# Quyans/GOI-Hyperplane

Hardware: AMD Instinct MI355X
Metric: training views/sec (rasterizer fwd+bwd), 1M Gaussians @1600x1056 RGB+16-d feat (higher is better)
Workload: dtype f32

## Files before the change

### goi_hyperplane_amd/_C.py

```python
from __future__ import annotations

import collections
import ctypes as C
import os
import threading
import warnings
import weakref

import torch

from . import _lib
from ._lib import ALLOC_FN, GoiRasterScene


_EXT = {"mod": None, "tried": False, "want": os.environ.get("GOI_BINDING", "compiled").strip().lower()}
_EMPTY = torch.Tensor([])


def _ext():
    if _EXT.get("error") is not None:
        raise _EXT["error"]
    if not _EXT["tried"]:
        _EXT["tried"] = True
        path = os.path.join(os.path.dirname(_lib.LIB_PATH), "_goi_C.so")
# ... 756 lines not shown
        alloc = _BinningAllocator(dev)
        n = lib.goi_raster_forward(C.byref(sc), _ptr(geom), _ptr(img), alloc.cb, None, _ptr(out_color), _ptr(out_sem),
                                   _ptr(out_depth), _ptr(out_alpha), _ptr(radii), _stream(dev))
        if alloc.error is not None:
            raise alloc.error
        if n < 0:
            raise RuntimeError(_lib.last_error())
        if P > 0:
            SPECULATION_STATS["exact_frames"] += 1
            _note_count(dev, P, n, _tiles(H, W))
    return n, out_color, out_sem, out_depth, out_alpha, radii, geom, alloc.tensor, img


def _backward_impl(background, means3D, radii, colors, semantics, scales, rotations, scale_modifier,
                                 cov3D_precomp, viewmatrix, projmatrix, tan_fovx, tan_fovy, dL_dout_color,
                                 dL_dout_semantic, dL_dout_depth, dL_dout_alpha, sh, degree, campos, geomBuffer, R,
                                 binningBuffer, imageBuffer, alphas, debug, sh_factored=False, accumulate_into=None):
    lib = _lib.load()
    dev = _check_device(means3D)
    ext = _ext()
    if ext is not None:
        R_layout, lazy_binning = _layout_of(R)
        return ext.backward_ex(background, means3D, radii, _e(colors), semantics, _e(scales), _e(rotations),
                               float(scale_modifier), _e(cov3D_precomp), viewmatrix, projmatrix, float(tan_fovx),
                               float(tan_fovy), dL_dout_color, dL_dout_semantic, dL_dout_depth, dL_dout_alpha, _e(sh),
                               int(degree), campos, geomBuffer, R_layout,
                               binningBuffer if lazy_binning is None else lazy_binning, imageBuffer, alphas, bool(debug),
                               bool(sh_factored), _scratch_instances(R, R_layout), accumulate_into)
    if accumulate_into is not None:
        raise RuntimeError("accumulate_into needs the compiled binding (python -m goi_hyperplane_amd.build)")
    P = int(means3D.size(0))
    H, W = int(alphas.size(-2)), int(alphas.size(-1))
    S = int(semantics.size(1))
    M = 0 if (sh is None or sh.numel() == 0) else int(sh.size(1))
    sh_factored = bool(sh_factored) and M > 0
    f32 = dict(dtype=torch.float32, device=dev)
    with torch.cuda.device(dev):
        sections = (("means3D", (P, 3)), ("sh", (P, 0 if sh_factored else M, 3)), ("semantics", (P, S)),
                    ("opacity", (P, 1)), ("scales", (P, 3)), ("rotations", (P, 4)))
        offs, total = {}, 0
        for name, shape in sections:
            offs[name] = total
            n = 1
            for d in shape:
                n *= d
            total += (n + 63) // 64 * 64
        flat = torch.empty((total,), **f32)

        def view(name, shape):
            n = 1
            for d in shape:
                n *= d
            return flat[offs[name]:offs[name] + n].view(shape)
        dL_dmeans3D = view("means3D", (P, 3))
        dL_dsh = None if sh_factored else view("sh", (P, M, 3))
        dL_dsemantics = view("semantics", (P, S))
        dL_dopacity = view("opacity", (P, 1))
        dL_dscales = view("scales", (P, 3))
        dL_drotations = view("rotations", (P, 4))
        del flat
        dL_dmeans2D = torch.empty((P, 3), **f32)
        dL_dcolors = torch.empty((P, 3), **f32)
        dL_ddepths = torch.empty((P, 1), **f32)
        dL_dconic = torch.empty((P, 2, 2), **f32)
        dL_dcov3D = torch.empty((P, 6), **f32)
        if P != 0:
            ten = dict(bg=_prep(background, "background", dev), means3D=_prep(means3D, "means3D", dev),
                       sh=_prep(sh, "sh", dev), colors=_prep(colors, "colors_precomp", dev),
                       semantics=_prep(semantics, "semantics", dev), scales=_prep(scales, "scales", dev),
                       rotations=_prep(rotations, "rotations", dev), cov3D=_prep(cov3D_precomp, "cov3D_precomp", dev),
                       viewmatrix=_prep(viewmatrix, "viewmatrix", dev), projmatrix=_prep(projmatrix, "projmatrix", dev),
                       campos=_prep(campos, "campos", dev), radii=_prep(radii, "radii", dev, torch.int32),
                       alphas=_prep(alphas, "alphas", dev), g_c=_prep(dL_dout_color, "dL_dout_color", dev),
                       g_s=_prep(dL_dout_semantic, "dL_dout_semantic", dev),
                       g_d=_prep(dL_dout_depth, "dL_dout_depth", dev), g_a=_prep(dL_dout_alpha, "dL_dout_alpha", dev))
            sc = _scene(P, S, H, W, ten["bg"], ten["means3D"], ten["sh"], ten["colors"], ten["semantics"], None,
                        ten["scales"], ten["rotations"], scale_modifier, ten["cov3D"], ten["viewmatrix"],
                        ten["projmatrix"], tan_fovx, tan_fovy, degree, ten["campos"], False, debug)
            R_layout, lazy_binning = _layout_of(R)
            if lazy_binning is not None:
                binningBuffer = lazy_binning
            R_scratch = _scratch_instances(R, R_layout)
            scratch = _backward_scratch(lib.goi_raster_backward_scratch_bytes(R_scratch or R_layout, S), dev)
            r = lib.goi_raster_backward3(
                C.byref(sc), R_layout, R_scratch, 0, _ptr(geomBuffer), _ptr(binningBuffer), _ptr(imageBuffer), _ptr(ten["radii"]),
                _ptr(ten["alphas"]), _ptr(ten["g_c"]), _ptr(ten["g_s"]), _ptr(ten["g_d"]), _ptr(ten["g_a"]),
                _ptr(dL_dmeans2D), _ptr(dL_dconic), _ptr(dL_dopacity), _ptr(dL_dcolors), _ptr(dL_dsemantics),
                _ptr(dL_ddepths), _ptr(dL_dmeans3D), _ptr(dL_dcov3D), _ptr(dL_dsh), _ptr(dL_dscales),
                _ptr(dL_drotations), _ptr(scratch), None, _stream(dev))
            if r < 0:
                raise RuntimeError(_lib.last_error())
    return (dL_dmeans2D, dL_dcolors, dL_dsemantics, dL_dopacity, dL_dmeans3D, dL_dcov3D, dL_dsh, dL_dscales,
            dL_drotations)


def rasterize_gaussians_backward(background, means3D, radii, colors, semantics, scales, rotations, scale_modifier,
                                 cov3D_precomp, viewmatrix, projmatrix, tan_fovx, tan_fovy, dL_dout_color,
                                 dL_dout_semantic, dL_dout_depth, dL_dout_alpha, sh, degree, campos, geomBuffer, R,
                                 binningBuffer, imageBuffer, alphas, debug):
    return _backward_impl(background, means3D, radii, colors, semantics, scales, rotations, scale_modifier, cov3D_precomp, viewmatrix, projmatrix, tan_fovx, tan_fovy, dL_dout_color, dL_dout_semantic, dL_dout_depth, dL_dout_alpha, sh, degree, campos, geomBuffer, R, binningBuffer, imageBuffer, alphas, debug)


def rasterize_gaussians_backward_accumulate(accumulate_into, *args):
    return _backward_impl(*args, accumulate_into=accumulate_into)


def rasterize_gaussians_backward_sh_factored(background, means3D, radii, colors, semantics, scales, rotations, scale_modifier,
                                 cov3D_precomp, viewmatrix, projmatrix, tan_fovx, tan_fovy, dL_dout_color,
                                 dL_dout_semantic, dL_dout_depth, dL_dout_alpha, sh, degree, campos, geomBuffer, R,
                                 binningBuffer, imageBuffer, alphas, debug):
    return _backward_impl(background, means3D, radii, colors, semantics, scales, rotations, scale_modifier, cov3D_precomp, viewmatrix, projmatrix, tan_fovx, tan_fovy, dL_dout_color, dL_dout_semantic, dL_dout_depth, dL_dout_alpha, sh, degree, campos, geomBuffer, R, binningBuffer, imageBuffer, alphas, debug, sh_factored=True)


def sh_grad_from_views(means3D, campos, gcol, degree, M):
    lib = _lib.load()
    dev = _check_device(means3D)
    P, V = int(means3D.size(0)), int(campos.size(0))
    if tuple(gcol.shape) != (V, P, 3):
        raise ValueError(f"gcol must be [V={V}, P={P}, 3], got {tuple(gcol.shape)}")
    with torch.cuda.device(dev):
        out = torch.empty((P, int(M), 3), dtype=torch.float32, device=dev)
        if P and V:
            m, c, g = _prep(means3D, "means3D", dev), _prep(campos, "campos", dev), _prep(gcol, "gcol", dev)
            if lib.goi_raster_sh_grad_from_views(P, int(degree), int(M), V, _ptr(m), _ptr(c), _ptr(g), _ptr(out), _stream(dev)) < 0:
                raise RuntimeError(_lib.last_error())
        elif P:
            out.zero_()
    return out


def rasterize_gaussians_backward_semantics(background, means3D, radii, semantics, viewmatrix, projmatrix, tan_fovx,
                                           tan_fovy, dL_dout_semantic, campos, geomBuffer, R, binningBuffer,
                                           imageBuffer, alphas, sh_degree=0, debug=False):
    lib = _lib.load()
    dev = _check_device(means3D)
    ext = _ext()
    if ext is not None:
        R_layout, lazy_binning = _layout_of(R)
        return ext.backward_semantics(background, means3D, radii, semantics, viewmatrix, projmatrix, float(tan_fovx),
                                      float(tan_fovy), dL_dout_semantic, campos, geomBuffer, R_layout,
                                      binningBuffer if lazy_binning is None else lazy_binning, imageBuffer, alphas,
                                      int(sh_degree), bool(debug))
    P = int(means3D.size(0))
    S = int(dL_dout_semantic.size(0))
    H, W = int(dL_dout_semantic.size(1)), int(dL_dout_semantic.size(2))
    with torch.cuda.device(dev):
        dL_dsemantics = torch.empty((P, S), dtype=torch.float32, device=dev)
        if P != 0:
            ten = dict(bg=_prep(background, "background", dev), means3D=_prep(means3D, "means3D", dev),
                       semantics=_prep(semantics, "semantics", dev), viewmatrix=_prep(viewmatrix, "viewmatrix", dev),
                       projmatrix=_prep(projmatrix, "projmatrix", dev), campos=_prep(campos, "campos", dev),
                       radii=_prep(radii, "radii", dev, torch.int32), alphas=_prep(alphas, "alphas", dev),
                       g_s=_prep(dL_dout_semantic, "dL_dout_semantic", dev))
            sc = _scene(P, S, H, W, ten["bg"], ten["means3D"], None, ten["means3D"], ten["semantics"], None,
                        None, None, 1.0, ten["means3D"], ten["viewmatrix"], ten["projmatrix"], tan_fovx, tan_fovy,
                        sh_degree, ten["campos"], False, debug)
            R_layout, lazy_binning = _layout_of(R)
            if lazy_binning is not None:
                binningBuffer = lazy_binning
            scratch = _backward_scratch(lib.goi_raster_backward_scratch_bytes(R_layout, S), dev)
            r = lib.goi_raster_backward_semantics(C.byref(sc), R_layout, _ptr(geomBuffer), _ptr(binningBuffer),
                                                  _ptr(imageBuffer), _ptr(ten["radii"]), _ptr(ten["alphas"]),
                                                  _ptr(ten["g_s"]), _ptr(dL_dsemantics), _ptr(scratch), _stream(dev))
            if r < 0:
                raise RuntimeError(_lib.last_error())
    return dL_dsemantics


def rasterize_gaussians_trace(background, means3D, colors, img_sem, opacity, scales, rotations, scale_modifier,
                              cov3D_precomp, viewmatrix, projmatrix, tan_fovx, tan_fovy, image_height, image_width, sh,
                              degree, campos, prefiltered, debug):
    lib = _lib.load()
# ... 115 lines not shown
```

### goi_hyperplane_amd/_lib.py

```python
from __future__ import annotations

import ctypes as C
import os

_HERE = os.path.dirname(os.path.abspath(__file__))
LIB_PATH = os.path.join(_HERE, "lib", "libgoi_raster.so")

ABI_VERSION = 6

STAGES = ("preprocess", "depth_sort", "scan", "emit", "tile_sort", "ranges", "blend_fwd", "blend_bwd",
          "preprocess_bwd")


class GoiRasterScene(C.Structure):
    _fields_ = [
        ("P", C.c_int), ("D", C.c_int), ("M", C.c_int), ("S", C.c_int), ("W", C.c_int), ("H", C.c_int),
        ("bg", C.c_void_p), ("means3D", C.c_void_p), ("shs", C.c_void_p), ("colors_precomp", C.c_void_p),
        ("semantics", C.c_void_p), ("opacities", C.c_void_p), ("scales", C.c_void_p),
        ("scale_modifier", C.c_float), ("rotations", C.c_void_p), ("cov3D_precomp", C.c_void_p),
        ("viewmatrix", C.c_void_p), ("projmatrix", C.c_void_p), ("campos", C.c_void_p),
        ("tan_fovx", C.c_float), ("tan_fovy", C.c_float), ("prefiltered", C.c_int), ("debug", C.c_int),
    ]


ALLOC_FN = C.CFUNCTYPE(C.c_void_p, C.c_void_p, C.c_size_t)

SYMBOLS = {
    "goi_raster_abi_version": (C.c_int, []),
    "goi_raster_last_error": (C.c_char_p, []),
    "goi_raster_geom_bytes": (C.c_size_t, [C.c_int]),
    "goi_raster_image_bytes": (C.c_size_t, [C.c_int, C.c_int]),
    "goi_raster_binning_bytes": (C.c_size_t, [C.c_int]),
    "goi_raster_backward_scratch_bytes": (C.c_size_t, [C.c_int, C.c_int]),
    "goi_raster_forward": (C.c_int, [C.POINTER(GoiRasterScene), C.c_void_p, C.c_void_p, ALLOC_FN, C.c_void_p]
                           + [C.c_void_p] * 5 + [C.c_void_p]),
    "goi_raster_forward_async": (C.c_int, [C.POINTER(GoiRasterScene), C.c_void_p, C.c_void_p, C.c_void_p, C.c_int]
                                 + [C.c_void_p] * 5 + [C.c_void_p]),
    "goi_raster_ticket_result": (C.c_int, [C.c_int, C.c_int, C.POINTER(C.c_int)]),
    "goi_raster_forward_async_cut": (C.c_int, [C.POINTER(GoiRasterScene), C.c_void_p, C.c_void_p, C.c_void_p, C.c_int]
                                     + [C.c_void_p] * 5 + [C.c_void_p, C.c_void_p, C.c_void_p]),
    "goi_raster_ticket_result2": (C.c_int, [C.c_int, C.c_int, C.POINTER(C.c_int), C.POINTER(C.c_uint)]),
    "goi_raster_forward_redo": (C.c_int, [C.POINTER(GoiRasterScene), C.c_int, C.c_void_p, C.c_void_p, C.c_void_p]
                                + [C.c_void_p] * 5 + [C.c_void_p]),
    "goi_raster_forward_reblend": (C.c_int, [C.POINTER(GoiRasterScene), C.c_int] + [C.c_void_p] * 9),
    "goi_raster_backward": (C.c_int, [C.POINTER(GoiRasterScene), C.c_int] + [C.c_void_p] * 3 + [C.c_void_p] * 6
                            + [C.c_void_p] * 11 + [C.c_void_p, C.c_void_p]),
    "goi_raster_backward2": (C.c_int, [C.POINTER(GoiRasterScene), C.c_int] + [C.c_void_p] * 3 + [C.c_void_p] * 6
                             + [C.c_void_p] * 11 + [C.c_void_p, C.c_void_p, C.c_void_p]),
    "goi_raster_backward3": (C.c_int, [C.POINTER(GoiRasterScene), C.c_int, C.c_int, C.c_int] + [C.c_void_p] * 3 + [C.c_void_p] * 6
                             + [C.c_void_p] * 11 + [C.c_void_p, C.c_void_p, C.c_void_p]),
    "goi_raster_backward_semantics": (C.c_int, [C.POINTER(GoiRasterScene), C.c_int] + [C.c_void_p] * 9),
    "goi_raster_trace": (C.c_int, [C.POINTER(GoiRasterScene), C.c_void_p, C.c_void_p, C.c_void_p, ALLOC_FN,
                                   C.c_void_p] + [C.c_void_p] * 4 + [C.c_void_p]),
    "goi_raster_mark_visible": (C.c_int, [C.c_int] + [C.c_void_p] * 4 + [C.c_void_p]),
    "goi_codebook_loss_partial_rows": (C.c_int, []),
    "goi_codebook_loss_rows": (C.c_int, [C.c_void_p] * 5 + [C.c_longlong, C.c_int, C.c_int, C.c_float] + [C.c_void_p] * 4),
    "goi_codebook_sim_workspace_bytes": (C.c_size_t, []),
    "goi_codebook_sim": (C.c_int, [C.c_void_p, C.c_void_p, C.c_longlong, C.c_int, C.c_int, C.c_void_p, C.c_void_p, C.c_void_p,
                                   C.c_void_p]),
    "goi_codebook_dlut_partial_blocks": (C.c_int, []),
    "goi_codebook_dlut": (C.c_int, [C.c_void_p, C.c_void_p, C.c_longlong, C.c_int, C.c_int, C.c_void_p, C.c_void_p]),
    "goi_codebook_fused_workspace_bytes": (C.c_size_t, [C.c_longlong]),
    "goi_codebook_fused_partial_rows": (C.c_int, []),
    "goi_codebook_fused": (C.c_int, [C.c_void_p] * 5 + [C.c_longlong, C.c_int, C.c_int, C.c_int, C.c_float] + [C.c_void_p] * 5),
    "goi_adam_step": (C.c_int, [C.c_void_p, C.c_int, C.c_double, C.c_double, C.c_double, C.c_void_p, C.c_void_p]),
    "goi_adam_step_guarded": (C.c_int, [C.c_void_p, C.c_int, C.c_double, C.c_double, C.c_double, C.c_void_p, C.c_void_p,
                                        C.c_void_p]),
    "goi_raster_truncated_flag": (C.c_void_p, [C.c_void_p, C.c_int]),
    "goi_knn_workspace_bytes": (C.c_size_t, [C.c_int]),
    "goi_knn_dist2": (C.c_int, [C.c_int, C.c_void_p, C.c_void_p, C.c_void_p, C.c_void_p]),
    "goi_raster_sh_grad_from_views": (C.c_int, [C.c_int, C.c_int, C.c_int, C.c_int, C.c_void_p, C.c_void_p, C.c_void_p, C.c_void_p,
                                        C.c_void_p]),
    "goi_raster_profile_enable": (None, [C.c_int]),
    "goi_raster_profile_stages": (None, [C.c_uint]),
    "goi_raster_profile_collect": (C.c_int, [C.POINTER(C.c_double), C.POINTER(C.c_int)]),
    "goi_semantic_decode": (C.c_int, [C.c_void_p, C.c_int, C.c_longlong, C.c_void_p, C.c_void_p, C.c_int, C.c_void_p,
                                      C.c_float, C.c_void_p, C.c_void_p, C.c_void_p, C.c_void_p]),
    "goi_semantic_osh_counts": (C.c_int, [C.c_void_p, C.c_void_p, C.c_longlong, C.c_int, C.c_void_p, C.c_void_p]),
    "goi_semantic_osh_fit": (C.c_int, [C.c_void_p, C.c_int, C.c_int, C.c_void_p, C.c_longlong, C.c_int, C.c_void_p, C.c_void_p,
                                       C.c_float, C.c_int, C.c_double] + [C.c_void_p] * 6),
    "goi_semantic_dbscan_workspace_bytes": (C.c_size_t, [C.c_longlong]),
    "goi_semantic_dbscan": (C.c_int, [C.c_longlong, C.c_void_p, C.c_float, C.c_int, C.c_void_p, C.c_void_p, C.c_void_p, C.c_void_p,
                                      C.c_void_p]),
    "goi_semantic_mask_pack": (C.c_int, [C.c_void_p, C.c_int, C.c_int, C.c_int, C.c_int, C.c_int, C.c_void_p, C.c_void_p, C.c_void_p]),
    "goi_semantic_mask_dilate": (C.c_int, [C.c_void_p, C.c_void_p, C.c_int, C.c_int, C.c_int, C.c_int, C.c_void_p]),
    "goi_semantic_mask_unpack": (C.c_int, [C.c_void_p] + [C.c_int] * 4 + [C.c_void_p] * 3),
    "goi_semantic_mask_confusion": (C.c_int, [C.c_void_p, C.c_void_p, C.c_int, C.c_int, C.c_int, C.c_void_p, C.c_void_p]),
    "goi_codebook_unique_rows_workspace_bytes": (C.c_size_t, [C.c_int] * 4),
    "goi_codebook_unique_rows": (C.c_int, [C.c_void_p] + [C.c_int] * 4 + [C.POINTER(C.c_longlong), C.POINTER(C.c_uint), ALLOC_FN,
                                           C.c_void_p, C.c_void_p, C.c_void_p]),
    "goi_codebook_kmeans_workspace_bytes": (C.c_size_t, [C.c_longlong, C.c_int, C.c_int, C.c_int]),
    "goi_codebook_kmeans": (C.c_int, [C.c_void_p, C.c_void_p, C.c_int, C.c_longlong, C.c_longlong] + [C.c_int] * 3
                            + [C.c_void_p] * 5),
    "goi_raster_photometric_workspace_bytes": (C.c_size_t, [C.c_longlong, C.c_int, C.c_int, C.c_int, C.c_uint]),
    "goi_raster_photometric_forward": (C.c_int, [C.c_void_p, C.c_void_p, C.c_longlong, C.c_int, C.c_int, C.c_int, C.c_int, C.c_float,
                                          C.c_uint] + [C.c_void_p] * 4),
    "goi_raster_photometric_backward": (C.c_int, [C.c_void_p, C.c_void_p, C.c_longlong, C.c_int, C.c_int, C.c_int, C.c_int, C.c_float,
                                           C.c_uint] + [C.c_void_p] * 5),
    "goi_raster_densify_workspace_bytes": (C.c_size_t, [C.c_longlong]),
    "goi_raster_densify_stats": (C.c_int, [C.c_longlong, C.c_void_p, C.c_longlong] + [C.c_void_p] * 4),
    "goi_raster_densify_plan": (C.c_int, [C.c_longlong] + [C.c_void_p] * 4 + [C.c_double] * 3 + [C.c_int, C.c_double, C.c_double]
                                + [C.c_void_p] * 3),
    "goi_raster_densify_prune_plan": (C.c_int, [C.c_longlong] + [C.c_void_p] * 4),
    "goi_raster_densify_apply": (C.c_int, [C.c_longlong, C.c_void_p, C.c_int] + [C.c_void_p] * 3 + [C.c_longlong, C.c_longlong]
                                 + [C.c_void_p] * 2),
    "goi_raster_set_option": (C.c_int, [C.c_char_p, C.c_int]),
    "goi_raster_blend_stats": (C.c_int, [C.c_int] * 4 + [C.c_void_p] * 5),
    "goi_raster_debug_views": (C.c_int, [C.c_int] * 4 + [C.c_void_p] * 3 + [C.c_void_p] * 8 + [C.c_void_p]),
    "goi_raster_debug_sort_workspace_bytes": (C.c_size_t, [C.c_longlong, C.c_int, C.c_int]),
    "goi_raster_debug_sort_pairs": (C.c_int, [C.c_void_p] * 4 + [C.c_longlong, C.c_int, C.c_int, C.c_void_p, C.c_void_p, C.c_int]
                                    + [C.c_void_p] * 3),
    "goi_raster_debug_scan_workspace_bytes": (C.c_size_t, [C.c_longlong]),
    "goi_raster_debug_exclusive_scan": (C.c_int, [C.c_void_p] * 3 + [C.c_longlong] + [C.c_void_p] * 4),
    "goi_raster_debug_reduce_row_floats": (C.c_int, [C.c_int, C.c_int]),
    "goi_raster_debug_reduce_workspace_bytes": (C.c_size_t, [C.c_longlong]),
    "goi_raster_debug_reduce_rows": (C.c_int, [C.c_int, C.c_int, C.c_int, C.c_longlong] + [C.c_void_p] * 14),
    "goi_raster_debug_preprocess_backward": (C.c_int, [C.POINTER(GoiRasterScene), C.c_int, C.c_int, C.c_int, C.c_longlong]
                                             + [C.c_void_p] * 22),
    "goi_raster_debug_pair_eval": (C.c_int, [C.c_int, C.c_int, C.c_int, C.c_void_p, C.c_void_p, C.c_longlong] + [C.c_void_p] * 4),
    "goi_raster_debug_backward_blend": (C.c_int, [C.POINTER(GoiRasterScene), C.c_int, C.c_int] + [C.c_void_p] * 24),
}

_lib = None


def load():
    global _lib
    if _lib is None:
        if not os.path.exists(LIB_PATH):
            raise ImportError(
                f"{LIB_PATH} is missing: the HIP extension has not been built. Run "
                "`python -m goi_hyperplane_amd.build` (needs hipcc; cross-compiles for gfx950 without a GPU). "
                "There is deliberately no CPU fallback.")
# ... 62 lines not shown
```

### goi_hyperplane_amd/csrc/api.hip

```cpp
#include <climits>
#include <cmath>
#include <cstdio>
#include <cstring>
#include <cstdlib>
#include <atomic>
#include <chrono>
#include <mutex>
#include <thread>
#include <string>
#include <vector>

#include "common.h"

namespace goi {

namespace {

thread_local std::string g_err;

int fail(const char* where, hipError_t e) {
    g_err = std::string(where) + ": " + hipGetErrorString(e);
    return -1;
}
int fail(const std::string& msg) {
// ... 295 lines not shown
    if (ticket < 0) return -1;
    const uint32_t* order = nullptr;
    if (enqueue_front(sc, g, im, radii, ticket, &order, s)) {
        ticket_release(ticket);
        return -1;
    }
    long long n64 = 0;
    if (ticket_result(ticket, 1, &n64) < 0) return -1;
    const int N = (int)n64;
    const size_t need = goi_raster_binning_bytes(N);
    char* bin_mem = static_cast<char*>(alloc(user, need));
    if (!bin_mem && need > 0) return fail("binning allocation callback returned NULL");
    BinView bv;
    binning_layout(N, bin_mem, &bv);
    if (qmask) *qmask = bv.qmask;
    if (enqueue_back(sc, g, im, bv, N, true, order, radii, plist, s)) return -1;
    return N;
}

}

thread_local Options g_options;
static Options g_shared_options;
static std::mutex g_options_mu;
void refresh_options() {
    std::lock_guard<std::mutex> lk(g_options_mu);
    g_options = g_shared_options;
}

static int tile_sort_result_index(int W, int H, int N) {
    if (N <= 0) return 0;
    const int gx = (W + TILE - 1) / TILE, gy = (H + TILE - 1) / TILE;
    const int passes = (tile_key_bits((uint32_t)(gx * gy)) + 7) / 8;
    return passes & 1;
}

size_t geom_layout(int P, char* base, GeomView* v) {
    char* p = base;
    const size_t n = (size_t)(P > 0 ? P : 1);
    GeomView tmp;
    GeomView& g = v ? *v : tmp;
    carve(p, g.rec, n);
    carve(p, g.cov3D, 6 * n);
    carve(p, g.tiles_touched, n);
    carve(p, g.clamped, n);
    carve(p, g.sort_keys[0], n);
    carve(p, g.sort_keys[1], n);
    carve(p, g.sort_vals[0], n);
    carve(p, g.sort_vals[1], n);
    g.bigq = g.sort_keys[1];
    carve(p, g.offsets, n);
    carve(p, g.aux, n);
    carve(p, g.blk_agg, (n + PRE_BLOCK - 1) / PRE_BLOCK);
    carve(p, g.blk_coarse, (((n + PRE_BLOCK - 1) / PRE_BLOCK + COARSE_BLOCKS - 1) / COARSE_BLOCKS) * (size_t)COARSE_STRIDE);
    carve(p, g.counters, COUNTER_WORDS);
    g.scratch_words = sort_scratch_words(n) + scan_scratch_words(n);
    carve(p, g.scratch, g.scratch_words);
    return (size_t)(p - base) + 256;
}

size_t image_layout(int W, int H, char* base, ImageView* v) {
    char* p = base;
    ImageView tmp;
    ImageView& im = v ? *v : tmp;
    const int gx = (W + TILE - 1) / TILE, gy = (H + TILE - 1) / TILE;
    carve(p, im.n_contrib, (size_t)W * H);
    carve(p, im.ranges, (size_t)gx * gy);
    carve(p, im.qcost, (size_t)gx * gy * 4);
    carve(p, im.qorder, (size_t)gx * gy * 4 + 8);
    carve(p, im.qmask0, (size_t)gx * gy * 4);
    return (size_t)(p - base) + 256;
}

size_t bwd_scratch_layout(int N, int S, char* base, BwdScratchView* v) {
    char* p = base;
    const size_t n = (size_t)(N > 0 ? N : 1) * 4;
    BwdScratchView tmp;
    BwdScratchView& b = v ? *v : tmp;
    carve(p, b.rows, n * (size_t)bwd_row_floats(S));
    carve(p, b.flags, n);
    b.cap_big = reduce_cap_big(n / 4);
    carve(p, b.big_ctl, 8);
    carve(p, b.big_desc, b.cap_big);
    return (size_t)(p - base) + 256;
}

size_t binning_layout(int N, char* base, BinView* v) {
    char* p = base;
    const size_t n = (size_t)(N > 0 ? N : 1);
    BinView tmp;
    BinView& b = v ? *v : tmp;
    carve(p, b.keys[0], n);
    carve(p, b.keys[1], n);
    carve(p, b.vals[0], n);
    carve(p, b.vals[1], n);
    b.scratch_words = sort_scratch_words(n) + 8;
    carve(p, b.scratch, b.scratch_words);
    carve(p, b.qmask, 4 * (n / 64 + 2));
    return (size_t)(p - base) + 256;
}

}

using namespace goi;

extern "C" {

int goi_raster_abi_version(void) { return GOI_RASTER_ABI_VERSION; }
const char* goi_raster_last_error(void) { return g_err.c_str(); }

size_t goi_raster_geom_bytes(int P) { return geom_layout(P, nullptr, nullptr) + 256; }
size_t goi_raster_image_bytes(int W, int H) { return image_layout(W, H, nullptr, nullptr) + 256; }
size_t goi_raster_binning_bytes(int N) { return binning_layout(N, nullptr, nullptr) + 256; }
size_t goi_raster_backward_scratch_bytes(int N, int S) { return bwd_scratch_layout(N, S, nullptr, nullptr) + 256; }

int goi_raster_forward(const GoiRasterScene* scene, void* geom_buffer, void* image_buffer, goi_alloc_fn binning_alloc,
                       void* alloc_user, float* out_color, float* out_semantic, float* out_depth, float* out_alpha,
                       int* radii, void* stream) {
    refresh_options();
    if (validate(scene, true)) return -1;
    const GoiRasterScene& sc = *scene;
    hipStream_t s = static_cast<hipStream_t>(stream);
    const size_t HW = (size_t)sc.W * sc.H;
    if (sc.P == 0) {
        GOI_HIP(hipMemsetAsync(out_color, 0, 3 * HW * sizeof(float), s));
        GOI_HIP(hipMemsetAsync(out_semantic, 0, (size_t)sc.S * HW * sizeof(float), s));
        GOI_HIP(hipMemsetAsync(out_depth, 0, HW * sizeof(float), s));
        GOI_HIP(hipMemsetAsync(out_alpha, 0, HW * sizeof(float), s));
        return 0;
    }
    if (!geom_buffer || !image_buffer || !binning_alloc) return fail("workspace pointer / allocator is NULL");
    GeomView g;
    ImageView im;
    geom_layout(sc.P, static_cast<char*>(geom_buffer), &g);
    image_layout(sc.W, sc.H, static_cast<char*>(image_buffer), &im);
    const uint32_t* plist = nullptr;
    unsigned long long* qmask = nullptr;
    const int N = geometry_and_binning(sc, g, im, binning_alloc, alloc_user, radii, &plist, s, &qmask);
    if (N < 0) return -1;
    {
        StageTimer t(GOI_STAGE_BLEND_FWD, s);
        launch_render_fwd(sc, g, im, plist, out_color, out_semantic, out_depth, out_alpha, s, qmask);
    }
    if (check_stage(sc, s, "forward blend")) return -1;
    GOI_HIP(hipGetLastError());
    return N;
}

int goi_raster_forward_async(const GoiRasterScene* scene, void* geom_buffer, void* image_buffer, void* binning_buffer,
                             int capacity, float* out_color, float* out_semantic, float* out_depth, float* out_alpha,
                             int* radii, void* stream) {
    return goi_raster_forward_async_cut(scene, geom_buffer, image_buffer, binning_buffer, capacity, out_color, out_semantic,
                                        out_depth, out_alpha, radii, nullptr, nullptr, stream);
}

int goi_raster_forward_async_cut(const GoiRasterScene* scene, void* geom_buffer, void* image_buffer, void* binning_buffer,
                                 int capacity, float* out_color, float* out_semantic, float* out_depth, float* out_alpha,
                                 int* radii, const float* zcut_in, float* zcut_out, void* stream) {
    refresh_options();
    if (validate(scene, true)) return -1;
    const GoiRasterScene& sc = *scene;
    hipStream_t s = static_cast<hipStream_t>(stream);
    if (sc.P == 0) return fail("goi_raster_forward_async: P == 0 has nothing to speculate on; use goi_raster_forward");
    if (sc.debug) return fail("goi_raster_forward_async: debug mode synchronises after every stage; use goi_raster_forward");
    if (g_options.sort_variant != 1) return fail("goi_raster_forward_async needs the onesweep sort (sort_variant 1)");
    if (capacity <= 0) return fail("goi_raster_forward_async: capacity must be positive");
    if (!geom_buffer || !image_buffer || !binning_buffer) return fail("workspace pointer is NULL");
    GeomView g;
    ImageView im;
    BinView bv;
    geom_layout(sc.P, static_cast<char*>(geom_buffer), &g);
    image_layout(sc.W, sc.H, static_cast<char*>(image_buffer), &im);
    binning_layout(capacity, static_cast<char*>(binning_buffer), &bv);
    const int ticket = ticket_acquire(capacity);
    if (ticket < 0) return -1;
    const uint32_t* order = nullptr;
    const uint32_t* plist = nullptr;
    uint32_t* zlearn = reinterpret_cast<uint32_t*>(zcut_out);
    if (enqueue_front(sc, g, im, radii, -1, &order, s, zcut_in, zlearn) ||
        enqueue_back(sc, g, im, bv, capacity, false, order, radii, &plist, s)) {
        ticket_release(ticket);
        return -1;
    }
    uint32_t* host_words = nullptr;
    uint32_t stamp = 0;
    {
        std::lock_guard<std::mutex> lk(g_ticket_mu);
        Ticket& tk = g_tickets[ticket];
        if (!zlearn && !zcut_in && tk.pinned_dev) {
            host_words = tk.pinned_dev;
            tk.seq = tk.seq + 1u ? tk.seq + 1u : 1u;
            stamp = tk.seq;
            tk.head_only = true;
            tk.stamped = true;
            tk.stream = s;
        }
    }
// ... 53 lines not shown
        StageTimer t(GOI_STAGE_BLEND_FWD, s);
        launch_render_fwd(sc, g, im, plist, out_color, out_semantic, out_depth, out_alpha, s, bv.qmask);
    }
    GOI_HIP(hipGetLastError());
    return 0;
}

int goi_raster_forward_reblend(const GoiRasterScene* scene, int R, const void* geom_buffer, const void* binning_buffer,
                               const void* cached_image_buffer, void* image_buffer, float* out_color, float* out_semantic,
                               float* out_depth, float* out_alpha, void* stream) {
    refresh_options();
    if (!scene) return fail("scene is NULL");
    const GoiRasterScene& sc = *scene;
    if (sc.P <= 0 || sc.W <= 0 || sc.H <= 0 || sc.S < 1 || sc.S > 32) return fail("goi_raster_forward_reblend: bad P/W/H/S");
    if (!sc.semantics || !sc.bg) return fail("goi_raster_forward_reblend: semantics and bg are required");
    if (R < 0) return fail("goi_raster_forward_reblend: bad R");
    if (!geom_buffer || !cached_image_buffer || !image_buffer || (R > 0 && !binning_buffer))
        return fail("workspace pointer is NULL");
    if (!out_color || !out_semantic || !out_depth || !out_alpha) return fail("output pointer is NULL");
    hipStream_t s = static_cast<hipStream_t>(stream);
    GeomView g;
    ImageView im_old, im;
    BinView bv;
    geom_layout(sc.P, static_cast<char*>(const_cast<void*>(geom_buffer)), &g);
    image_layout(sc.W, sc.H, static_cast<char*>(const_cast<void*>(cached_image_buffer)), &im_old);
    image_layout(sc.W, sc.H, static_cast<char*>(image_buffer), &im);
    binning_layout(R, static_cast<char*>(const_cast<void*>(binning_buffer)), &bv);
    const int gx = (sc.W + TILE - 1) / TILE, gy = (sc.H + TILE - 1) / TILE;
    GOI_HIP(hipMemcpyAsync(im.ranges, im_old.ranges, sizeof(uint2) * (size_t)gx * gy, hipMemcpyDeviceToDevice, s));
    const uint32_t* plist = bv.vals[tile_sort_result_index(sc.W, sc.H, R)];
    {
        StageTimer t(GOI_STAGE_BLEND_FWD, s);
        launch_render_fwd(sc, g, im, plist, out_color, out_semantic, out_depth, out_alpha, s, bv.qmask);
    }
    GOI_HIP(hipGetLastError());
    return 0;
}

int goi_raster_trace(const GoiRasterScene* scene, const float* img_sem, void* geom_buffer, void* image_buffer,
                     goi_alloc_fn binning_alloc, void* alloc_user, float* out_color, float* gau_sem, int* num_gsem,
                     int* radii, void* stream) {
    refresh_options();
    if (validate(scene, false)) return -1;
    const GoiRasterScene& sc = *scene;
    hipStream_t s = static_cast<hipStream_t>(stream);
    const size_t HW = (size_t)sc.W * sc.H;
    GOI_HIP(hipMemsetAsync(out_color, 0, 3 * HW * sizeof(float), s));
    if (sc.P == 0) return 0;
    if (!img_sem) return fail("img_sem is NULL");
    if (!geom_buffer || !image_buffer || !binning_alloc) return fail("workspace pointer / allocator is NULL");
    GOI_HIP(hipMemsetAsync(gau_sem, 0, (size_t)sc.P * sc.S * sizeof(float), s));
    GOI_HIP(hipMemsetAsync(num_gsem, 0, (size_t)sc.P * sizeof(int), s));
    GeomView g;
    ImageView im;
    geom_layout(sc.P, static_cast<char*>(geom_buffer), &g);
    image_layout(sc.W, sc.H, static_cast<char*>(image_buffer), &im);
    const uint32_t* plist = nullptr;
    const int N = geometry_and_binning(sc, g, im, binning_alloc, alloc_user, radii, &plist, s);
    if (N < 0) return -1;
    launch_trace_fwd(sc, img_sem, g, im, plist, out_color, gau_sem, num_gsem, s);
    if (check_stage(sc, s, "trace")) return -1;
    GOI_HIP(hipGetLastError());
    return N;
}

int goi_raster_backward(const GoiRasterScene* scene, int R, const void* geom_buffer, const void* binning_buffer,
                        const void* image_buffer, const int* radii, const float* out_alpha, const float* dL_dout_color,
                        const float* dL_dout_semantic, const float* dL_dout_depth, const float* dL_dout_alpha,
                        float* dL_dmean2D, float* dL_dconic, float* dL_dopacity, float* dL_dcolor, float* dL_dsemantic,
                        float* dL_ddepth, float* dL_dmean3D, float* dL_dcov3D, float* dL_dsh, float* dL_dscale,
                        float* dL_drot, void* scratch, void* stream) {
    return goi_raster_backward2(scene, R, geom_buffer, binning_buffer, image_buffer, radii, out_alpha, dL_dout_color,
                                dL_dout_semantic, dL_dout_depth, dL_dout_alpha, dL_dmean2D, dL_dconic, dL_dopacity, dL_dcolor,
                                dL_dsemantic, dL_ddepth, dL_dmean3D, dL_dcov3D, dL_dsh, dL_dscale, dL_drot, scratch, nullptr,
                                stream);
}

int goi_raster_backward3(const GoiRasterScene* scene, int R, int scratch_instances, int flags, const void* geom_buffer,
                         const void* binning_buffer, const void* image_buffer, const int* radii, const float* out_alpha,
                         const float* dL_dout_color, const float* dL_dout_semantic, const float* dL_dout_depth,
                         const float* dL_dout_alpha, float* dL_dmean2D, float* dL_dconic, float* dL_dopacity, float* dL_dcolor,
                         float* dL_dsemantic, float* dL_ddepth, float* dL_dmean3D, float* dL_dcov3D, float* dL_dsh,
                         float* dL_dscale, float* dL_drot, void* scratch, const int* prev_radii, void* stream) {
    refresh_options();
    if (validate(scene, true, false)) return -1;
    const GoiRasterScene& sc = *scene;
    hipStream_t s = static_cast<hipStream_t>(stream);
    const size_t P = (size_t)sc.P;
    if (P == 0) return 0;
    if (!geom_buffer || !image_buffer || (R > 0 && !binning_buffer)) return fail("workspace pointer is NULL");
    GeomView g;
    ImageView im;
    BinView bv;
    geom_layout(sc.P, const_cast<char*>(static_cast<const char*>(geom_buffer)), &g);
    image_layout(sc.W, sc.H, const_cast<char*>(static_cast<const char*>(image_buffer)), &im);
    const int fin = tile_sort_result_index(sc.W, sc.H, R);
    if (R > 0) binning_layout(R, const_cast<char*>(static_cast<const char*>(binning_buffer)), &bv);
    const bool rows_path = scratch != nullptr && (g_options.bwd_variant & 15) != 1;
    if (scratch_instances < 0 || scratch_instances > R) return fail("scratch_instances must be in 0..R (0: the scratch is laid out for R)");
    const int Rs = scratch_instances > 0 ? scratch_instances : R;
    const bool accumulate = (flags & GOI_BACKWARD_ACCUMULATE) != 0;
    if (accumulate && (!rows_path || g_options.bwd_records != 1 || prev_radii || (sc.shs && !dL_dsh) || sc.debug))
        return fail("GOI_BACKWARD_ACCUMULATE needs the default backward (scratch given, bwd_variant 0 / 2, bwd_records 1), dL_dsh when "
                    "the colours are SH, prev_radii NULL and debug off");
    if (rows_path) {
        BwdScratchView scr;
        bwd_scratch_layout(Rs, sc.S, static_cast<char*>(scratch), &scr);
        {
            StageTimer t(GOI_STAGE_BLEND_BWD, s);
            if (R > 0) {
                if (!launch_quad_order(sc, im, s, scr.flags, g.counters + COUNTER_N, (uint32_t)Rs, scr.big_ctl)) {
                    GOI_HIP(hipMemsetAsync(scr.flags, 0, round_up_256((size_t)Rs * 4), s));
                    GOI_HIP(hipMemsetAsync(scr.big_ctl, 0, 8 * sizeof(uint32_t), s));
                }
                launch_render_bwd_rows(sc, g, im, bv.vals[fin], radii, out_alpha, dL_dout_color, dL_dout_semantic,
                                       dL_dout_depth, dL_dout_alpha, scr, s, bv.qmask);
            }
        }
        if (check_stage(sc, s, "backward blend")) return -1;
        StageTimer t(GOI_STAGE_PREPROCESS_BWD, s);
        if (g_options.bwd_records == 2 && bwd_row_floats(sc.S) == 32 && R > 0 && !accumulate) {
            launch_reduce_big_only(sc, g, Rs, scr, s);
            launch_preprocess_bwd(sc, g, radii, dL_dmean2D, dL_dconic, dL_dcolor, dL_ddepth, dL_dmean3D, dL_dcov3D, dL_dsh,
                                  dL_dscale, dL_drot, s, scr.rows, dL_dopacity, dL_dsemantic, prev_radii, scr.flags, Rs);
        } else if (g_options.bwd_records) {
            launch_reduce_rows(sc, g, Rs, scr, nullptr, nullptr, nullptr, nullptr, nullptr, nullptr, s, true);
            launch_preprocess_bwd(sc, g, radii, dL_dmean2D, dL_dconic, dL_dcolor, dL_ddepth, dL_dmean3D, dL_dcov3D, dL_dsh,
                                  dL_dscale, dL_drot, s, scr.rows, dL_dopacity, dL_dsemantic, prev_radii, nullptr, 0, accumulate);
        } else {
            launch_reduce_rows(sc, g, Rs, scr, dL_dmean2D, dL_dconic, dL_dopacity, dL_dcolor, dL_dsemantic, dL_ddepth, s);
            launch_preprocess_bwd(sc, g, radii, dL_dmean2D, dL_dconic, dL_dcolor, dL_ddepth, dL_dmean3D, dL_dcov3D, dL_dsh,
                                  dL_dscale, dL_drot, s);
        }
    } else {
        GOI_HIP(hipMemsetAsync(dL_dmean2D, 0, 3 * P * sizeof(float), s));
        GOI_HIP(hipMemsetAsync(dL_dconic, 0, 4 * P * sizeof(float), s));
        GOI_HIP(hipMemsetAsync(dL_dopacity, 0, P * sizeof(float), s));
        GOI_HIP(hipMemsetAsync(dL_dcolor, 0, 3 * P * sizeof(float), s));
        GOI_HIP(hipMemsetAsync(dL_dsemantic, 0, (size_t)sc.S * P * sizeof(float), s));
        GOI_HIP(hipMemsetAsync(dL_ddepth, 0, P * sizeof(float), s));
        if (R > 0) {
            StageTimer t(GOI_STAGE_BLEND_BWD, s);
            launch_render_bwd_tile(sc, g, im, bv.vals[fin], out_alpha, dL_dout_color, dL_dout_semantic, dL_dout_depth,
                                   dL_dout_alpha, dL_dmean2D, dL_dconic, dL_dopacity, dL_dcolor, dL_dsemantic,
                                   dL_ddepth, s);
        }
        if (check_stage(sc, s, "backward blend")) return -1;
        StageTimer t(GOI_STAGE_PREPROCESS_BWD, s);
        launch_preprocess_bwd(sc, g, radii, dL_dmean2D, dL_dconic, dL_dcolor, dL_ddepth, dL_dmean3D, dL_dcov3D, dL_dsh,
                              dL_dscale, dL_drot, s);
    }
    if (check_stage(sc, s, "backward preprocess")) return -1;
    GOI_HIP(hipGetLastError());
    return 0;
}

int goi_raster_backward2(const GoiRasterScene* scene, int R, const void* geom_buffer, const void* binning_buffer,
                         const void* image_buffer, const int* radii, const float* out_alpha, const float* dL_dout_color,
                         const float* dL_dout_semantic, const float* dL_dout_depth, const float* dL_dout_alpha,
                         float* dL_dmean2D, float* dL_dconic, float* dL_dopacity, float* dL_dcolor, float* dL_dsemantic,
                         float* dL_ddepth, float* dL_dmean3D, float* dL_dcov3D, float* dL_dsh, float* dL_dscale,
                         float* dL_drot, void* scratch, const int* prev_radii, void* stream) {
    return goi_raster_backward3(scene, R, 0, 0, geom_buffer, binning_buffer, image_buffer, radii, out_alpha, dL_dout_color,
                                dL_dout_semantic, dL_dout_depth, dL_dout_alpha, dL_dmean2D, dL_dconic, dL_dopacity, dL_dcolor,
                                dL_dsemantic, dL_ddepth, dL_dmean3D, dL_dcov3D, dL_dsh, dL_dscale, dL_drot, scratch, prev_radii,
                                stream);
}

int goi_raster_backward_semantics(const GoiRasterScene* scene, int R, const void* geom_buffer, const void* binning_buffer,
                                  const void* image_buffer, const int* radii, const float* out_alpha,
                                  const float* dL_dout_semantic, float* dL_dsemantic, void* scratch, void* stream) {
    refresh_options();
    if (validate(scene, true, false)) return -1;
    const GoiRasterScene& sc = *scene;
    hipStream_t s = static_cast<hipStream_t>(stream);
    if (sc.P == 0) return 0;
    if (!geom_buffer || !image_buffer || (R > 0 && !binning_buffer)) return fail("workspace pointer is NULL");
    if (!scratch) return fail("goi_raster_backward_semantics needs the scratch of goi_raster_backward_scratch_bytes");
    if (!dL_dout_semantic || !dL_dsemantic || !out_alpha || !radii) return fail("a required pointer is NULL");
    GeomView g;
    ImageView im;
    BinView bv;
    geom_layout(sc.P, const_cast<char*>(static_cast<const char*>(geom_buffer)), &g);
    image_layout(sc.W, sc.H, const_cast<char*>(static_cast<const char*>(image_buffer)), &im);
    const int fin = tile_sort_result_index(sc.W, sc.H, R);
    if (R > 0) binning_layout(R, const_cast<char*>(static_cast<const char*>(binning_buffer)), &bv);
    BwdScratchView scr;
    bwd_scratch_layout(R, sc.S, static_cast<char*>(scratch), &scr);
    const int row_floats = bwd_sem_row_floats(sc.S);
    {
        StageTimer t(GOI_STAGE_BLEND_BWD, s);
        if (R > 0) {
            if (!launch_quad_order(sc, im, s, scr.flags, g.counters + COUNTER_N, (uint32_t)R, scr.big_ctl)) {
                GOI_HIP(hipMemsetAsync(scr.flags, 0, round_up_256((size_t)R * 4), s));
                GOI_HIP(hipMemsetAsync(scr.big_ctl, 0, 8 * sizeof(uint32_t), s));
            }
            launch_render_bwd_sem(sc, g, im, bv.vals[fin], radii, out_alpha, dL_dout_semantic, scr.rows, scr.flags,
                                  row_floats, s, bv.qmask);
        }
    }
    if (check_stage(sc, s, "backward blend (semantics)")) return -1;
    StageTimer t(GOI_STAGE_PREPROCESS_BWD, s);
    launch_reduce_sem_rows(sc, g, R, scr, row_floats, dL_dsemantic, s);
    GOI_HIP(hipGetLastError());
    return 0;
}

int goi_raster_mark_visible(int P, const float* means3D, const float* viewmatrix, const float* projmatrix,
                            uint8_t* present, void* stream) {
    (void)projmatrix;
    if (P < 0) return fail("bad P");
    if (P == 0) return 0;
    if (!means3D || !viewmatrix || !present) return fail("NULL pointer");
    launch_mark_visible(P, means3D, viewmatrix, present, static_cast<hipStream_t>(stream));
    GOI_HIP(hipGetLastError());
    return 0;
}

int goi_semantic_decode(const float* sem, int S, long long HW, const float* W, const float* bias, int n_codes,
                        const float* code_score, float thresh, float* sim_out, int* idx_out, uint8_t* bg_mask_out,
                        void* stream) {
    refresh_options();
    if (!sem || !W || !bias) return fail("goi_semantic_decode: NULL input");
    if (S < 1 || S > 32 || n_codes < 1 || HW < 0) return fail("goi_semantic_decode: need 1 <= S <= 32, n_codes >= 1");
    if (HW == 0) return 0;
    if (launch_semantic_decode(sem, S, HW, W, bias, n_codes, code_score, thresh, sim_out, idx_out, bg_mask_out,
                               static_cast<hipStream_t>(stream)) < 0)
        return fail("goi_semantic_decode: code book too large for LDS");
    GOI_HIP(hipGetLastError());
    return 0;
}

int goi_semantic_osh_counts(const int* idx, const uint8_t* positive, long long HW, int n_codes, int* counts, void* stream) {
// ... 353 lines not shown
    if (P <= 0 || V <= 0) return 0;
    if (D < 0 || D > 3 || M < (D + 1) * (D + 1) || M > 16) return fail("goi_raster_sh_grad_from_views: need 0 <= D <= 3 and (D+1)^2 <= M <= 16");
    if (!means3D || !campos || !gcol || !dL_dsh) return fail("goi_raster_sh_grad_from_views: NULL pointer");
    launch_sh_grad_from_views(P, D, M, V, means3D, campos, gcol, dL_dsh, static_cast<hipStream_t>(stream));
    if (hipGetLastError() != hipSuccess) return fail("goi_raster_sh_grad_from_views: launch failed");
    return 0;
}

int goi_adam_step(const GoiAdamGroup* groups, int n_groups, double beta1, double beta2, double eps,
                  const unsigned char* nograd_mask, void* stream) {
    return goi_adam_step_guarded(groups, n_groups, beta1, beta2, eps, nograd_mask, nullptr, stream);
}

const uint32_t* goi_raster_truncated_flag(const void* geom_buffer, int P) {
    if (!geom_buffer || P <= 0) return nullptr;
    GeomView g;
    geom_layout(P, const_cast<char*>(static_cast<const char*>(geom_buffer)), &g);
    return g.counters + COUNTER_OVF;
}

int goi_adam_step_guarded(const GoiAdamGroup* groups, int n_groups, double beta1, double beta2, double eps,
                          const unsigned char* nograd_mask, const uint32_t* skip_flag, void* stream) {
    if (n_groups < 0 || n_groups > GOI_ADAM_MAX_GROUPS) return fail("goi_adam_step: n_groups must be 0..8");
    if (n_groups && !groups) return fail("goi_adam_step: groups is NULL");
    for (int i = 0; i < n_groups; i++) {
        const GoiAdamGroup& g = groups[i];
        if (g.numel < 0 || g.row_len < 1) return fail("goi_adam_step: bad numel / row_len");
        if (g.numel == 0) continue;
        if (!g.param || !g.grad || !g.exp_avg || !g.exp_avg_sq) return fail("goi_adam_step: a tensor pointer is NULL");
        if ((reinterpret_cast<uintptr_t>(g.param) | reinterpret_cast<uintptr_t>(g.grad) |
             reinterpret_cast<uintptr_t>(g.exp_avg) | reinterpret_cast<uintptr_t>(g.exp_avg_sq)) & 15)
            return fail("goi_adam_step: tensors must be 16-byte aligned");
    }
    launch_adam_step(groups, n_groups, beta1, beta2, eps, nograd_mask, skip_flag, static_cast<hipStream_t>(stream));
    GOI_HIP(hipGetLastError());
    return 0;
}

size_t goi_knn_workspace_bytes(int P) { return P > 0 && P < SORT_MAX_KEYS ? knn_workspace_bytes(P) : 0; }

int goi_knn_dist2(int P, const float* points, float* mean_dist2, void* workspace, void* stream) {
    if (P < 0) return fail("goi_knn_dist2: bad P");
    if (P >= SORT_MAX_KEYS) return fail("goi_knn_dist2: need P < 2^30");
    if (P == 0) return 0;
    if (!points || !mean_dist2 || !workspace) return fail("goi_knn_dist2: a required pointer is NULL");
    if (reinterpret_cast<uintptr_t>(workspace) & 255) return fail("goi_knn_dist2: workspace must be 256-byte aligned");
    launch_knn(P, points, mean_dist2, workspace, static_cast<hipStream_t>(stream));
    GOI_HIP(hipGetLastError());
    return 0;
}

void goi_raster_profile_enable(int on) { g_profile_mask.store(on ? ~0u : 0u); }

void goi_raster_profile_stages(unsigned stage_mask) { g_profile_mask.store(stage_mask); }

int goi_raster_set_option(const char* name, int value) {
    if (!name) return fail("option name is NULL");
    std::lock_guard<std::mutex> lk(g_options_mu);
    Options& g_options = g_shared_options;
    if (!strcmp(name, "fwd_variant")) {
        if (value < 0 || value > 1) return fail("fwd_variant must be 0 or 1");
        g_options.fwd_variant = value;
    }
    else if (!strcmp(name, "bwd_variant")) {
        if (value < 0 || value > 2) return fail("bwd_variant must be 0, 1 or 2");
        g_options.bwd_variant = value;
    }
    else if (!strcmp(name, "sort_variant")) g_options.sort_variant = value;
    else if (!strcmp(name, "sort_small")) g_options.sort_small = value;
    else if (!strcmp(name, "sort_lookback")) g_options.sort_lookback = value;
    else if (!strcmp(name, "cull_variant")) g_options.cull_variant = value;
    else if (!strcmp(name, "bwd_order")) {
        if (value < 0 || value > 8) return fail("bwd_order must be 0 .. 8");
        g_options.bwd_order = value;
    }
    else if (!strcmp(name, "decode_variant")) g_options.decode_variant = value;
    else if (!strcmp(name, "bwd_masks")) {
        if (value < 0 || value > 1) return fail("bwd_masks must be 0 or 1");
        g_options.bwd_masks = value;
    }
    else if (!strcmp(name, "bwd_records")) {
        if (value < 0 || value > 2) return fail("bwd_records must be 0, 1 or 2");
        g_options.bwd_records = value;
    }
    else if (!strcmp(name, "osh_path")) {
        if (value < 0 || value > 1) return fail("osh_path must be 0 or 1");
        g_options.osh_path = value;
    }
    else return fail(std::string("unknown option ") + name);
    return 0;
}

int goi_raster_profile_collect(double* ms, int* calls) {
    std::vector<StageEvents> events;
    {
        std::lock_guard<std::mutex> lk(g_profile_mu);
        events.swap(g_events);
    }
    for (auto& ev : events) {
        GOI_HIP(hipEventSynchronize(ev.b));
        float t = 0.f;
        GOI_HIP(hipEventElapsedTime(&t, ev.a, ev.b));
        if (ms) ms[ev.stage] += (double)t;
        if (calls) calls[ev.stage] += 1;
        std::lock_guard<std::mutex> lk(g_profile_mu);
        g_pool.push_back(ev.a);
        g_pool.push_back(ev.b);
    }
    return 0;
}

int goi_raster_blend_stats(int P, int W, int H, int R, const void* geom_buffer, const void* binning_buffer,
                           const void* image_buffer, unsigned long long* counters, void* stream) {
    hipStream_t s = static_cast<hipStream_t>(stream);
    if (P <= 0 || W <= 0 || H <= 0 || R < 0) return fail("goi_raster_blend_stats: bad P/W/H/R");
    if (!geom_buffer || !image_buffer || !counters || (R > 0 && !binning_buffer)) return fail("workspace pointer is NULL");
    GOI_HIP(hipMemsetAsync(counters, 0, GOI_BLEND_STATS_WORDS * sizeof(unsigned long long), s));
    if (R == 0) return 0;
    GeomView g;
    ImageView im;
    BinView bv;
    geom_layout(P, const_cast<char*>(static_cast<const char*>(geom_buffer)), &g);
    image_layout(W, H, const_cast<char*>(static_cast<const char*>(image_buffer)), &im);
    binning_layout(R, const_cast<char*>(static_cast<const char*>(binning_buffer)), &bv);
    launch_blend_stats(W, H, g, im, bv.vals[tile_sort_result_index(W, H, R)], bv.qmask, counters, s);
    GOI_HIP(hipGetLastError());
    return 0;
}

int goi_raster_debug_views(int P, int W, int H, int R, const void* geom_buffer, const void* binning_buffer,
                           const void* image_buffer, float* depths, float* means2D, float* conic_opacity, float* rgb,
                           uint32_t* tiles_touched, uint32_t* point_list, uint32_t* ranges, uint32_t* n_contrib,
                           void* stream) {
    hipStream_t s = static_cast<hipStream_t>(stream);
    if (P <= 0) return 0;
    GeomView g;
    ImageView im;
    geom_layout(P, const_cast<char*>(static_cast<const char*>(geom_buffer)), &g);
    image_layout(W, H, const_cast<char*>(static_cast<const char*>(image_buffer)), &im);
    const int gx = (W + TILE - 1) / TILE, gy = (H + TILE - 1) / TILE;
    const char* rec = reinterpret_cast<const char*>(g.rec);
    const size_t pitch = sizeof(GaussRec);
    if (means2D) GOI_HIP(hipMemcpy2DAsync(means2D, 8, rec + 0, pitch, 8, P, hipMemcpyDeviceToDevice, s));
    if (conic_opacity) {
        GOI_HIP(hipMemcpy2DAsync(conic_opacity, 16, rec + 8, pitch, 8, P, hipMemcpyDeviceToDevice, s));
        GOI_HIP(hipMemcpy2DAsync(reinterpret_cast<char*>(conic_opacity) + 8, 16, rec + 16, pitch, 8, P,
                                 hipMemcpyDeviceToDevice, s));
    }
    if (depths) GOI_HIP(hipMemcpy2DAsync(depths, 4, rec + 44, pitch, 4, P, hipMemcpyDeviceToDevice, s));
    if (rgb) GOI_HIP(hipMemcpy2DAsync(rgb, 12, rec + 32, pitch, 12, P, hipMemcpyDeviceToDevice, s));
    if (tiles_touched)
        GOI_HIP(hipMemcpyAsync(tiles_touched, g.tiles_touched, sizeof(uint32_t) * P, hipMemcpyDeviceToDevice, s));
    if (ranges) GOI_HIP(hipMemcpyAsync(ranges, im.ranges, sizeof(uint2) * gx * gy, hipMemcpyDeviceToDevice, s));
    if (n_contrib)
        GOI_HIP(hipMemcpyAsync(n_contrib, im.n_contrib, sizeof(uint32_t) * (size_t)W * H, hipMemcpyDeviceToDevice, s));
    if (point_list && R > 0) {
        BinView bv;
        binning_layout(R, const_cast<char*>(static_cast<const char*>(binning_buffer)), &bv);
        const int fin = tile_sort_result_index(W, H, R);
        GOI_HIP(hipMemcpyAsync(point_list, bv.vals[fin], sizeof(uint32_t) * (size_t)R, hipMemcpyDeviceToDevice, s));
    }
    return 0;
}

static int debug_sort_args(const char* fn, long long n, int lo, int hi) {
    if (n < 0 || n >= SORT_MAX_KEYS) return fail(std::string(fn) + ": need 0 <= n < 2^30");
// ... 302 lines not shown
```

### goi_hyperplane_amd/csrc/common.h

```cpp
#pragma once

#include <hip/hip_runtime.h>
#include <stddef.h>
#include <stdint.h>

#include "goi_raster.h"

namespace goi {

constexpr int TILE = 16;
constexpr int TILE_PIX = TILE * TILE;
constexpr int WAVE = 64;

struct GaussRec {
    float4 q0, q1, q2;
};

struct GeomView {
    GaussRec* rec;
    float* cov3D;
    uint32_t* tiles_touched;
    uint8_t* clamped;
    uint32_t* sort_keys[2];
    uint32_t* sort_vals[2];
    uint32_t* offsets;
    uint4* aux;
    uint2* blk_agg;
    unsigned long long* blk_coarse;
    uint32_t* bigq;
    uint32_t* scratch;
    uint32_t* counters;
    size_t scratch_words;
};
struct ImageView {
    uint32_t* n_contrib;
    uint2* ranges;
    uint32_t* qcost;
    uint32_t* qorder;
    unsigned long long* qmask0;
};
inline int bwd_row_floats(int S) { return ((4 * ((S + 3) / 4) + 4 + 6 + 15) / 16) * 16; }
inline int bwd_sem_row_floats(int S) { return ((4 * ((S + 3) / 4) + 15) / 16) * 16; }
#ifndef GOI_REDUCE_BIG_INST
#define GOI_REDUCE_BIG_INST 384
#endif
#ifndef GOI_REDUCE_HUGE_INST
#define GOI_REDUCE_HUGE_INST 2048
#endif
#ifndef GOI_REDUCE_DENSE_RATIO
#define GOI_REDUCE_DENSE_RATIO 10
#endif
constexpr uint32_t REDUCE_BIG_INST = GOI_REDUCE_BIG_INST, REDUCE_HUGE_INST = GOI_REDUCE_HUGE_INST,
                   REDUCE_DENSE_RATIO = GOI_REDUCE_DENSE_RATIO;
inline size_t reduce_cap_big(size_t n_cap) { return (n_cap > 0 ? n_cap : 1) / REDUCE_BIG_INST + 2; }
struct BwdScratchView {
    float* rows;
    uint8_t* flags;
    uint32_t* big_ctl;
    uint4* big_desc;
    size_t cap_big;
};
size_t bwd_scratch_layout(int N, int S, char* base, BwdScratchView* v);

struct BinView {
    uint32_t* keys[2];
    uint32_t* vals[2];
    uint32_t* scratch;
    size_t scratch_words;
    unsigned long long* qmask;
};

__host__ __device__ inline unsigned long long* member_mask_ptr(unsigned long long* qmask0, unsigned long long* qmask, int tile,
                                                                int q, uint32_t x0, int r) {
    return r == 0 ? qmask0 + ((size_t)tile * 4 + q) : qmask + (((size_t)(x0 >> 6) + (size_t)r) * 4 + q);
}

size_t geom_layout(int P, char* base, GeomView* v);
size_t image_layout(int W, int H, char* base, ImageView* v);
size_t binning_layout(int N, char* base, BinView* v);

struct Options {
    int fwd_variant = 1;
    int bwd_variant = 0;
    int sort_variant = 1;
    int sort_lookback = 1;
    int sort_small = 0;
    int decode_variant = 1;
    int cull_variant = 2;
    int bwd_order = 1;
    int bwd_masks = 1;
    int bwd_records = 1;
    int osh_path = 0;
};
extern thread_local Options g_options;
void refresh_options();

size_t scan_scratch_words(size_t n);
size_t sort_scratch_words(size_t n);
void exclusive_scan_u32(const uint32_t* in, const uint32_t* gather, uint32_t* out, size_t n, uint32_t* total,
                        uint32_t* scratch, hipStream_t s, const uint32_t* n_dev = nullptr);
int radix_sort_pairs(uint32_t* keys[2], uint32_t* vals[2], size_t n, int lo, int hi, uint32_t* scratch,
                     hipStream_t s, bool cleared = false, bool ghist_ready = false, const uint32_t* n_dev = nullptr,
                     uint32_t* frame_error = nullptr);
size_t radix_sort_control_words(size_t n, int lo, int hi);
uint32_t* radix_sort_ghist(uint32_t* scratch, size_t n, int lo, int hi);
void radix_sort_report_error(const uint32_t* scratch, size_t n, int lo, int hi, uint32_t* out, hipStream_t s);
constexpr long long SORT_MAX_KEYS = 1ll << 30;

void launch_preprocess_fwd(const GoiRasterScene& sc, const GeomView& g, int* radii, uint2* ranges, int n_tiles,
                           hipStream_t s, const float* zcut = nullptr, uint32_t* zlearn = nullptr);
void launch_compact_listed(int P, const GeomView& g, uint32_t* ghist, bool pad, hipStream_t s);
constexpr int COARSE_BLOCKS = 32, COARSE_STRIDE = 8;
constexpr int SORT_MAX_PASSES = 4, SORT_GH_COPIES = 8;
constexpr int PRE_BLOCK = 256;
void launch_emit(int P, int W, int H, const GeomView& g, const uint32_t* order, const int* radii, uint32_t* keys,
                 uint32_t* vals, uint32_t cap, hipStream_t s);
bool emit_can_count_tiles(int W, int H);
void launch_emit_counting(int P, int W, int H, const GeomView& g, const uint32_t* order, const int* radii, uint32_t* keys,
                          uint32_t* vals, uint2* ranges, uint32_t* clear, size_t clear_words, uint32_t cap, hipStream_t s);
void launch_tile_ranges_hist(int W, int H, uint2* ranges, uint32_t* ghist, uint32_t* counters, hipStream_t s);
void launch_ranges(int N, const uint32_t* n_dev, const uint32_t* sorted_keys, uint2* ranges, int T, hipStream_t s);
void launch_render_fwd(const GoiRasterScene& sc, const GeomView& g, const ImageView& im, const uint32_t* point_list,
                       float* out_color, float* out_sem, float* out_depth, float* out_alpha, hipStream_t s,
                       unsigned long long* qmask = nullptr, const float* zcut = nullptr, uint32_t* zlearn = nullptr,
                       uint32_t* host_words = nullptr,
                       uint32_t stamp = 0);
constexpr int HOST_STAMP_WORD = 33;
void launch_blend_stats(int W, int H, const GeomView& g, const ImageView& im, const uint32_t* point_list,
                        const unsigned long long* qmask, unsigned long long* out, hipStream_t s);
void launch_pair_eval(int P, int W, int H, const GeomView& g, const uint32_t* requests, long long n, float* E, float* alpha,
                      uint8_t* guards, hipStream_t s);
void launch_trace_fwd(const GoiRasterScene& sc, const float* img_sem, const GeomView& g, const ImageView& im,
                      const uint32_t* point_list, float* out_color, float* gau_sem, int* num_gsem, hipStream_t s);
bool quad_order_enabled(int W, int H);
bool launch_quad_order(const GoiRasterScene& sc, const ImageView& im, hipStream_t s, uint8_t* clear_flags = nullptr,
                       const uint32_t* n_dev = nullptr, uint32_t cap = 0, uint32_t* clear_ctl = nullptr);
void launch_render_bwd_rows(const GoiRasterScene& sc, const GeomView& g, const ImageView& im,
                            const uint32_t* point_list, const int* radii, const float* out_alpha, const float* dL_dpix,
                            const float* dL_dsem, const float* dL_ddepth, const float* dL_dalpha,
                            const BwdScratchView& scr, hipStream_t s, const unsigned long long* qmask = nullptr);
void launch_render_bwd_sem(const GoiRasterScene& sc, const GeomView& g, const ImageView& im, const uint32_t* point_list,
                           const int* radii, const float* out_alpha, const float* dL_dsem, float* rows, uint8_t* flags,
                           int row_floats, hipStream_t s, const unsigned long long* qmask = nullptr);
void launch_reduce_big_only(const GoiRasterScene& sc, const GeomView& g, int N, const BwdScratchView& scr, hipStream_t s);
void launch_reduce_sem_rows(const GoiRasterScene& sc, const GeomView& g, int N, const BwdScratchView& scr, int row_floats,
                            float* dL_dsemantic, hipStream_t s);
void launch_reduce_rows(const GoiRasterScene& sc, const GeomView& g, int N, const BwdScratchView& scr, float* dL_dmean2D,
                        float* dL_dconic, float* dL_dopacity, float* dL_dcolor, float* dL_dsemantic, float* dL_ddepth,
                        hipStream_t s, bool records = false);
void launch_render_bwd_tile(const GoiRasterScene& sc, const GeomView& g, const ImageView& im,
                            const uint32_t* point_list, const float* out_alpha, const float* dL_dpix,
                            const float* dL_dsem, const float* dL_ddepth, const float* dL_dalpha, float* dL_dmean2D,
                            float* dL_dconic, float* dL_dopacity, float* dL_dcolor, float* dL_dsemantic,
                            float* dL_ddepths, hipStream_t s);
void launch_sh_grad_from_views(int P, int D, int M, int V, const float* means3D, const float* campos, const float* gcol,
                               float* dL_dsh, hipStream_t s);
void launch_preprocess_bwd(const GoiRasterScene& sc, const GeomView& g, const int* radii, float* dL_dmean2D,
                           const float* dL_dconic, float* dL_dcolor, const float* dL_ddepth, float* dL_dmean3D,
                           float* dL_dcov3D, float* dL_dsh, float* dL_dscale, float* dL_drot, hipStream_t s,
                           const float* record_rows = nullptr, float* dL_dopacity = nullptr, float* dL_dsemantic = nullptr,
                           const int* prev_radii = nullptr,
                           const uint8_t* row_flags = nullptr, int N_cap = 0,
                           bool accumulate = false,
                           int max_blocks = 0);
int launch_semantic_decode(const float* sem, int S, long long HW, const float* W, const float* bias, int n_codes,
                           const float* code_score, float thresh, float* sim_out, int* idx_out, uint8_t* bg_mask_out,
                           hipStream_t s);
int codebook_loss_waves();
int launch_codebook_rows(const float* sim, const float* inv_gnorm, const float* sem, const float* W, const float* bias,
                         long long HW, int C, int S, float t, float* dsim, float* dsem, float* partials, hipStream_t s);
size_t codebook_sim_workspace_bytes();
int launch_codebook_sim(const float* g, const float* l1, long long HW, int C, int D, float* sim, float* inv_gnorm,
                        void* workspace, hipStream_t s);
int codebook_dlut_blocks();
size_t codebook_fused_workspace_bytes(long long HW);
int codebook_fused_rows();
int launch_codebook_fused(const float* g, const float* l1, const float* sem, const float* W, const float* bias, long long HW,
                          int C, int D, int S, float t, float* dsem, float* partials, float* dl1_partial, void* workspace,
                          hipStream_t s);
int launch_codebook_dlut(const float* dsim, const float* g, long long HW, int C, int D, float* partial, hipStream_t s);
int osh_max_codes();
int osh_max_dim();
bool osh_register_path(int n_codes, int D);
void launch_osh_counts(const int* idx, const uint8_t* positive, long long HW, int n_codes, int* counts, hipStream_t s);
void launch_osh_fit(const float* lut, int n_codes, int D, const int* counts, long long HW, int K, float* w, float* b,
                    float lr, int max_epochs, double target_iou, int* epochs_out, float* loss_out, double* iou_out,
                    double* init_iou_out, double* trace, hipStream_t s);
int launch_adam_step(const GoiAdamGroup* groups, int n_groups, double beta1, double beta2, double eps,
                     const uint8_t* nograd_mask, const uint32_t* skip_flag, hipStream_t s);
size_t knn_workspace_bytes(int P);
int launch_knn(int P, const float* points, float* mean_dist2, void* workspace, hipStream_t s);
size_t dbscan_workspace_bytes(size_t n);
void launch_dbscan(int n, const float* pts, float eps2, double h, int min_samples, int* labels, uint8_t* core, int* result,
                   void* workspace, hipStream_t s);
void launch_mask_pack(const void* src, int src_dtype, int n_views, int H, int W, int first_view, uint64_t* packed,
                      long long* counts, hipStream_t s);
void launch_mask_dilate(const uint64_t* src, uint64_t* dst, int n_views, int H, int W, int radius, hipStream_t s);
void launch_mask_unpack(const uint64_t* packed, int n_views, int H, int W, int n_out, const long long* index, uint8_t* out,
                        hipStream_t s);
void launch_mask_confusion(const uint64_t* pred, const uint64_t* gt, int n_views, int H, int W, long long* out, hipStream_t s);
size_t uniq_workspace_bytes(int V, int D, uint32_t HW);
uint32_t* uniq_counts(void* ws, int V, int D, uint32_t HW);
void launch_uniq_dedup(const float* const* maps, int V, int D, uint32_t HW, void* ws, hipStream_t s);
bool launch_uniq_sort(const float* map, int v, int V, int D, uint32_t HW, uint32_t N, float* out, void* ws, hipStream_t s);
size_t kmeans_workspace_bytes(long long rows, int K, int k, int D);
void launch_kmeans(float* x, const long long* off, int K, long long max_rows, long long total_rows, int D, int k, int niter,
                   const int* perms, float* centers, int* status, void* ws, hipStream_t s);
void launch_mark_visible(int P, const float* means3D, const float* view, uint8_t* present, hipStream_t s);
constexpr int PHOTO_RADIUS = GOI_PHOTOMETRIC_WINDOW / 2;
size_t photometric_workspace_bytes(long long n, int c, int h, int w, unsigned flags);
void launch_photometric_forward(const float* x, const float* y, long long n, int c, int h, int w, float lambda, unsigned flags,
                                float* out, float* out_images, void* ws, hipStream_t s);
void launch_photometric_backward(const float* x, const float* y, long long n, int c, int h, int w, float lambda, unsigned flags,
                                 const float* grad_out, const void* ws, float* gx, float* gy, hipStream_t s);

struct DensifyThresholds {
    float max_grad, thr_scale, min_opacity, big_world, split_inv;
    int screen, screen_all;
};
struct DensifyView {
    uint8_t* flags;
    uint32_t* rank;
    uint32_t* scratch;
    uint32_t* total;
};
size_t densify_layout(long long P, char* base, DensifyView* v);
void launch_densify_stats(long long P, const float* grad, long long stride, const uint8_t* filter, float* accum, float* denom,
                          hipStream_t s);
void launch_densify_plan(long long P, const float* accum, const float* denom, const float* scaling, const float* opacity,
                         const DensifyThresholds& t, uint32_t* counts, const DensifyView& v, hipStream_t s);
void launch_prune_plan(long long P, const uint8_t* mask, uint32_t* counts, const DensifyView& v, hipStream_t s);
void launch_densify_apply(long long P, const GoiDensifyRows* groups, int n_groups, const float* rotation, const float* scaling,
                          const float* z, long long n_split, long long kept_children, float split_inv, const DensifyView& v,
                          hipStream_t s);

__device__ __forceinline__ void tile_rect(float px, float py, int r, int gx, int gy, int& x0, int& y0, int& x1,
                                          int& y1) {
    x0 = min(gx, max(0, (int)((px - r) / TILE)));
    y0 = min(gy, max(0, (int)((py - r) / TILE)));
    x1 = min(gx, max(0, (int)((px + r + TILE - 1) / TILE)));
    y1 = min(gy, max(0, (int)((py + r + TILE - 1) / TILE)));
}

__device__ __forceinline__ void listed_rect(float px, float py, int r, float hx, float hy, bool cull, int gx, int gy,
                                            int& x0, int& y0, int& x1, int& y1) {
    tile_rect(px, py, r, gx, gy, x0, y0, x1, y1);
    if (!cull) return;
// ... 60 lines not shown
```

### goi_hyperplane_amd/csrc/preprocess.hip

```cpp
#include <algorithm>
#include <type_traits>

#include "common.h"
#include "gmath.h"
#include "row_sum.h"

namespace goi {

namespace {

__device__ __forceinline__ float ndc_to_pix(float v, int S) { return (float)(((v + 1.0) * S - 1.0) * 0.5); }

__device__ __forceinline__ M3 rotation_from_quat(float r, float x, float y, float z) {
    return make_m3(1.f - 2.f * (y * y + z * z), 2.f * (x * y - r * z), 2.f * (x * z + r * y),
                   2.f * (x * y + r * z), 1.f - 2.f * (x * x + z * z), 2.f * (y * z - r * x),
                   2.f * (x * z - r * y), 2.f * (y * z + r * x), 1.f - 2.f * (x * x + y * y));
}

struct Cov2D {
    M3 T, Vrk, W;
    V3 t;
    float txtz, tytz, limx, limy;
    M3 cov;
};
// ... 228 lines not shown
    }

    if (vis) {
        float4* r4 = reinterpret_cast<float4*>(rec + idx);
        r4[0] = make_float4(pix, piy, con_a, con_b);
        r4[1] = make_float4(con_c, o, hx, hy);
    }
    if (live) {
        radii[idx] = my_radius_i;
        tiles_touched[idx] = touched;
        raw_key[idx] = key;
        aux[idx] = make_uint4(0u, (uint32_t)my_radius_i, (uint32_t)tmask_v, (uint32_t)(tmask_v >> 32));
    }

    float cr = 0.f, cg = 0.f, cb = 0.f;
    V3 dir = {0.f, 0.f, 0.f};
    if (vis && !a.colors_precomp) {
        const V3 campos = {a.campos[0], a.campos[1], a.campos[2]};
        dir = p - campos;
        dir = dir / sqrtf(dot3(dir, dir));
    }
    auto finish_colour = [&](const V3& res) {
        clamp_bits = (uint8_t)((res.x < 0 ? 1 : 0) | (res.y < 0 ? 2 : 0) | (res.z < 0 ? 4 : 0));
        cr = fmaxf(res.x, 0.0f);
        cg = fmaxf(res.y, 0.0f);
        cb = fmaxf(res.z, 0.0f);
    };
    if (vis) {
        if (a.colors_precomp) {
            cr = a.colors_precomp[3 * idx];
            cg = a.colors_precomp[3 * idx + 1];
            cb = a.colors_precomp[3 * idx + 2];
        } else {
            float rowf[48];
            const bool row16 = a.M == 16;
            if (row16) {
                const float4* r4 = reinterpret_cast<const float4*>(a.shs + (size_t)idx * 48);
#pragma unroll
                for (int i = 0; i < 12; i++) {
                    const float4 v = r4[i];
                    rowf[4 * i] = v.x;
                    rowf[4 * i + 1] = v.y;
                    rowf[4 * i + 2] = v.z;
                    rowf[4 * i + 3] = v.w;
                }
            }
            const V3* shg = reinterpret_cast<const V3*>(a.shs) + (size_t)idx * a.M;
            finish_colour(sh_to_rgb_sum(a.D, dir, [&](int k) { return row16 ? V3{rowf[3 * k], rowf[3 * k + 1], rowf[3 * k + 2]} : shg[k]; }));
        }
    }
    if (vis) reinterpret_cast<float4*>(rec + idx)[2] = make_float4(cr, cg, cb, p_view.z);
    if (live) clamped[idx] = clamp_bits;
    __shared__ uint32_t s_wsum[4], s_wvis[4];
    uint32_t wsum = live ? touched : 0u;
#pragma unroll
    for (int d = 32; d >= 1; d >>= 1) wsum += (uint32_t)__shfl_xor((int)wsum, d, 64);
    const uint32_t wvis = (uint32_t)__popcll(__ballot(live && touched > 0));
    if ((threadIdx.x & 63) == 0) {
        s_wsum[threadIdx.x >> 6] = wsum;
        s_wvis[threadIdx.x >> 6] = wvis;
    }
    __syncthreads();
    if (threadIdx.x == 0) {
        const uint32_t bsum = s_wsum[0] + s_wsum[1] + s_wsum[2] + s_wsum[3];
        if (bsum) atomicAdd(&counters[NR_BASE + NR_STRIDE * (blockIdx.x % NR_STRIPES)], bsum);
        const uint32_t bvis = s_wvis[0] + s_wvis[1] + s_wvis[2] + s_wvis[3];
        blk_agg[blockIdx.x] = make_uint2(bvis, bsum);
        if (bvis) atomicAdd(&blk_coarse[(size_t)(blockIdx.x / COARSE_BLOCKS) * COARSE_STRIDE], ((unsigned long long)bvis << 40) | bsum);
    }
}

struct BwdArgs {
    int P, D, M, W, H;
    const float* means3D;
    const float* shs;
    const float* scales;
    const float* rotations;
    const float* cov3D;
    float scale_modifier, tan_fovx, tan_fovy, focal_x, focal_y;
    const float* view_p;
    const float* proj_p;
    const float* campos_p;
    const int* prev_radii;
    int accumulate;
};

struct RecArgs {
    const float* rows;
    const uint4* aux;
    const uint32_t* tiles_touched;
    int row_floats, S, nch;
    float* dL_dopacity;
    float* dL_dsemantic;
    const uint8_t* flags;
    const uint32_t* n_dev;
    uint32_t N_cap;
};
#ifndef GOI_PBWD_ROWS
#define GOI_PBWD_ROWS 224
#endif
#ifndef GOI_PBWD_BLOCKS
#define GOI_PBWD_BLOCKS 3
#endif
#ifndef GOI_PBWD_HOIST
#define GOI_PBWD_HOIST 1
#endif
constexpr int BWD_TILE_ROWS_DEFAULT = GOI_PBWD_ROWS;
#ifndef GOI_PBWD_INFLIGHT
#define GOI_PBWD_INFLIGHT 16
#endif
#ifndef GOI_PBWD_ROWS_FUSED
#define GOI_PBWD_ROWS_FUSED 208
#endif
constexpr int BWD_TILE_ROWS_FUSED = GOI_PBWD_ROWS_FUSED;
constexpr int BWD_REC_FLOATS = 10;
constexpr int BWD_BLOCKS_PER_CU = GOI_PBWD_BLOCKS;
constexpr bool BWD_HOIST = GOI_PBWD_HOIST != 0;

template <bool WITH_DSH, int SRC>
__global__ __launch_bounds__(256, GOI_PBWD_BLOCKS) void preprocess_bwd_k(const BwdArgs args, const int* __restrict__ radii,
                                                        const uint32_t* __restrict__ counters,
                                                        const uint8_t* __restrict__ clamped,
                                                        float* dL_dmean2D,
                                                        const float* __restrict__ dL_dconic,
                                                        float* dL_dcolor,
                                                        const float* __restrict__ dL_ddepth, const RecArgs ra,
                                                        float* __restrict__ dL_dmean3D, float* __restrict__ dL_dcov3D,
                                                        float* __restrict__ dL_dsh, float* __restrict__ dL_dscale,
                                                        float* __restrict__ dL_drot) {
    constexpr bool FROM_ROWS = SRC != 0;
    constexpr int BWD_TILE_ROWS = SRC == 2 ? BWD_TILE_ROWS_FUSED : BWD_TILE_ROWS_DEFAULT;
    extern __shared__ float s_dsh[];
    __shared__ uint32_t s_vis[BWD_TILE_ROWS + 256];
    __shared__ uint16_t s_zero[256];
    __shared__ uint32_t s_src[SRC == 1 ? BWD_TILE_ROWS : 1];
    __shared__ float s_rec[SRC == 2 ? BWD_TILE_ROWS * BWD_REC_FLOATS : 1];
    __shared__ int s_wcnt[2][4];
    const Camera cam = load_camera(args.view_p, args.proj_p, args.campos_p);
    struct : BwdArgs {
        const float *view, *proj, *campos;
    } a;
    static_cast<BwdArgs&>(a) = args;
    a.view = cam.view;
    a.proj = cam.proj;
    a.campos = cam.campos;
    const int w = 3 * a.M;
    const int nseg = (args.P + 255) / 256;
    const bool truncated = counters[COUNTER_OVF] != 0;
    int npend = 0;
    for (int seg = blockIdx.x; seg < nseg || npend > 0; seg += gridDim.x) {
    int nzero = 0;
    const int base = seg * 256;
    if (seg < nseg) {
        const int gtid = base + threadIdx.x;
        const bool live = gtid < args.P;
        const bool vis_t = live && radii[gtid] > 0 && !truncated;
        const bool keep_t = live && !vis_t && args.prev_radii != nullptr && args.prev_radii[gtid] == 0;
        const bool zero_t = live && !vis_t && !keep_t && !args.accumulate;
        const int wv = threadIdx.x >> 6;
        const unsigned long long bv = __ballot(vis_t), bz = __ballot(zero_t);
        if ((threadIdx.x & 63) == 0) {
            s_wcnt[0][wv] = __popcll(bv);
            s_wcnt[1][wv] = __popcll(bz);
        }
        __syncthreads();
        int ov = 0, oz = 0;
        for (int i = 0; i < wv; i++) {
            ov += s_wcnt[0][i];
            oz += s_wcnt[1][i];
        }
        const int nv = s_wcnt[0][0] + s_wcnt[0][1] + s_wcnt[0][2] + s_wcnt[0][3];
        nzero = s_wcnt[1][0] + s_wcnt[1][1] + s_wcnt[1][2] + s_wcnt[1][3];
        const unsigned long long lt = (1ull << (threadIdx.x & 63)) - 1ull;
        if (vis_t) s_vis[npend + ov + __popcll(bv & lt)] = (uint32_t)gtid;
        if (zero_t) s_zero[oz + __popcll(bz & lt)] = (uint16_t)threadIdx.x;
        npend += nv;
        __syncthreads();
    }
    if (nzero > 0) {
        if ((int)threadIdx.x < nzero) {
            const int idx = base + s_zero[threadIdx.x];
            if constexpr (FROM_ROWS) {
                ra.dL_dopacity[idx] = 0.f;
                dL_dmean2D[3 * idx] = dL_dmean2D[3 * idx + 1] = dL_dmean2D[3 * idx + 2] = 0.f;
                dL_dcolor[3 * idx] = dL_dcolor[3 * idx + 1] = dL_dcolor[3 * idx + 2] = 0.f;
            }
            dL_dmean3D[3 * idx] = dL_dmean3D[3 * idx + 1] = dL_dmean3D[3 * idx + 2] = 0.f;
#pragma unroll
            for (int i = 0; i < 6; i++) dL_dcov3D[(size_t)6 * idx + i] = 0.f;
            dL_dscale[3 * idx] = dL_dscale[3 * idx + 1] = dL_dscale[3 * idx + 2] = 0.f;
            reinterpret_cast<float4*>(dL_drot)[idx] = make_float4(0.f, 0.f, 0.f, 0.f);
        }
        if constexpr (FROM_ROWS) {
            for (int i = threadIdx.x; i < nzero * ra.S; i += 256) {
                const int r = i / ra.S;
                ra.dL_dsemantic[(size_t)(base + s_zero[r]) * ra.S + (i - r * ra.S)] = 0.f;
            }
        }
        if constexpr (WITH_DSH) {
            for (int i = threadIdx.x; i < nzero * w; i += 256) {
                const int r = i / w;
                dL_dsh[(size_t)(base + s_zero[r]) * w + (i - r * w)] = 0.f;
            }
        }
    }
    const bool last_trip = seg + (int)gridDim.x >= nseg;
    while (npend >= BWD_TILE_ROWS || (last_trip && npend > 0)) {
    const int nrows = min(BWD_TILE_ROWS, npend);
    const bool visible = (int)threadIdx.x < nrows;
    const int idx = visible ? (int)s_vis[threadIdx.x] : 0;
    if constexpr (WITH_DSH && BWD_HOIST) {
        if ((w & 3) == 0) {
            const int w4 = w >> 2;
            for (int i = threadIdx.x; i < nrows * w4; i += 256) {
                const int r = i / w4, q = i - r * w4;
                const float4 v = reinterpret_cast<const float4*>(a.shs + (size_t)s_vis[r] * w)[q];
                float* dst = s_dsh + r * (w + 1) + 4 * q;
                dst[0] = v.x;
                dst[1] = v.y;
                dst[2] = v.z;
                dst[3] = v.w;
            }
        } else {
            for (int i = threadIdx.x; i < nrows * w; i += 256) {
                const int r = i / w;
                s_dsh[r * (w + 1) + (i - r * w)] = a.shs[(size_t)s_vis[r] * w + (i - r * w)];
            }
        }
    }
    if constexpr (SRC == 2) {
        constexpr int RF = 32;
        const int qw = threadIdx.x >> 4, e = threadIdx.x & 15, quarter = (threadIdx.x & 63) >> 4;
        const uint32_t* flags32 = reinterpret_cast<const uint32_t*>(ra.flags);
        const uint32_t N = min(ra.N_cap, ra.n_dev[0]);
        const uint32_t Vl = ra.n_dev[COUNTER_V - COUNTER_N];
        const uint32_t big_inst = (N > REDUCE_DENSE_RATIO * Vl) ? REDUCE_BIG_INST : 1024u;
        const int rounds = (nrows + 15) >> 4;
        struct Meta {
            uint32_t idx, off0, cnt;
        };
        auto load_meta = [&](int k) {
            const int r = qw + 16 * k;
            Meta m{0u, 0u, 0u};
            if (k < rounds && r < nrows) {
                m.idx = s_vis[r];
                m.cnt = ra.tiles_touched[m.idx];
                m.off0 = ra.aux[m.idx].x;
                if (m.cnt == 0u) m.off0 = 0u;
            }
            return m;
        };
        auto load_first = [&](const Meta& m) { return (m.cnt <= big_inst && (uint32_t)e < m.cnt) ? flags32[m.off0 + e] : 0u; };
        Meta cur = load_meta(0), nxt = load_meta(1);
        uint32_t w_cur = load_first(cur);
#pragma unroll 1
        for (int k = 0; k < rounds; k++) {
            const Meta nn = load_meta(k + 2);
// ... 305 lines not shown
            const auto& A = dMt.c;
            grot.x = 2 * z * (A[0][1] - A[1][0]) + 2 * y * (A[2][0] - A[0][2]) + 2 * x * (A[1][2] - A[2][1]);
            grot.y = 2 * y * (A[1][0] + A[0][1]) + 2 * z * (A[2][0] + A[0][2]) + 2 * r * (A[1][2] - A[2][1]) -
                     4 * x * (A[2][2] + A[1][1]);
            grot.z = 2 * x * (A[1][0] + A[0][1]) + 2 * r * (A[2][0] - A[0][2]) + 2 * z * (A[1][2] + A[2][1]) -
                     4 * y * (A[2][2] + A[0][0]);
            grot.w = 2 * r * (A[0][1] - A[1][0]) + 2 * x * (A[2][0] + A[0][2]) + 2 * y * (A[1][2] + A[2][1]) -
                     4 * z * (A[1][1] + A[0][0]);
        }
    }
    if (visible) {
        if (a.accumulate) {
            const float m0 = dL_dmean3D[3 * idx], m1 = dL_dmean3D[3 * idx + 1], m2 = dL_dmean3D[3 * idx + 2];
            float c6[6];
#pragma unroll
            for (int i = 0; i < 6; i++) c6[i] = dL_dcov3D[(size_t)6 * idx + i];
            const float s0 = dL_dscale[3 * idx], s1 = dL_dscale[3 * idx + 1], s2 = dL_dscale[3 * idx + 2];
            const float4 r4 = reinterpret_cast<const float4*>(dL_drot)[idx];
            gmean = gmean + V3{m0, m1, m2};
#pragma unroll
            for (int i = 0; i < 6; i++) gcov[i] += c6[i];
            gscale = gscale + V3{s0, s1, s2};
            grot = make_float4(grot.x + r4.x, grot.y + r4.y, grot.z + r4.z, grot.w + r4.w);
        }
        dL_dmean3D[3 * idx] = gmean.x;
        dL_dmean3D[3 * idx + 1] = gmean.y;
        dL_dmean3D[3 * idx + 2] = gmean.z;
#pragma unroll
        for (int i = 0; i < 6; i++) dL_dcov3D[(size_t)6 * idx + i] = gcov[i];
        dL_dscale[3 * idx] = gscale.x;
        dL_dscale[3 * idx + 1] = gscale.y;
        dL_dscale[3 * idx + 2] = gscale.z;
        reinterpret_cast<float4*>(dL_drot)[idx] = grot;
    }
    if constexpr (WITH_DSH || FROM_ROWS) __syncthreads();
    if constexpr (SRC == 1) {
        if ((ra.S & 3) == 0) {
            const int S4 = ra.S >> 2;
            for (int i = threadIdx.x; i < nrows * S4; i += 256) {
                const int r = i / S4, sub = i - r * S4;
                const uint32_t o = s_src[r];
                const float4 v = o != 0xFFFFFFFFu ? *reinterpret_cast<const float4*>(ra.rows + (size_t)o * 4 * ra.row_floats + 4 * sub)
                                                  : make_float4(0.f, 0.f, 0.f, 0.f);
                float4* dst = reinterpret_cast<float4*>(ra.dL_dsemantic + (size_t)s_vis[r] * ra.S + 4 * sub);
                if (a.accumulate) {
                    const float4 p = *dst;
                    *dst = make_float4(p.x + v.x, p.y + v.y, p.z + v.z, p.w + v.w);
                } else {
                    *dst = v;
                }
            }
        } else {
            for (int i = threadIdx.x; i < nrows * ra.S; i += 256) {
                const int r = i / ra.S, ch = i - r * ra.S;
                const uint32_t o = s_src[r];
                const float v = o != 0xFFFFFFFFu ? ra.rows[(size_t)o * 4 * ra.row_floats + ch] : 0.f;
                float* dst = &ra.dL_dsemantic[(size_t)s_vis[r] * ra.S + ch];
                *dst = a.accumulate ? *dst + v : v;
            }
        }
    }
    if constexpr (WITH_DSH) {
        const int dr = 256 / w, dc = 256 - dr * w;
        int r = (int)threadIdx.x / w, col = (int)threadIdx.x - r * w;
        while (r < nrows) {
            float* dst = &dL_dsh[(size_t)s_vis[r] * w + col];
            *dst = a.accumulate ? *dst + s_dsh[r * (w + 1) + col] : s_dsh[r * (w + 1) + col];
            r += dr;
            col += dc;
            if (col >= w) {
                col -= w;
                r++;
            }
        }
    }
    __syncthreads();
    const int rest = npend - nrows;
    const uint32_t moved = (int)threadIdx.x < rest ? s_vis[nrows + threadIdx.x] : 0u;
    __syncthreads();
    if ((int)threadIdx.x < rest) s_vis[threadIdx.x] = moved;
    npend = rest;
    __syncthreads();
    }
    }
}

__global__ __launch_bounds__(256) void sh_grad_from_views_k(int P, int D, int M, int V, const float* __restrict__ means3D,
                                                            const float* __restrict__ campos,
                                                            const float* __restrict__ gcol,
                                                            float* __restrict__ dL_dsh) {
    extern __shared__ float s_dsh[];
    const int gtid = blockIdx.x * blockDim.x + threadIdx.x;
    const int idx = gtid < P ? gtid : P - 1;
    const V3 mean = {means3D[3 * idx], means3D[3 * idx + 1], means3D[3 * idx + 2]};
    V3 acc[16];
#pragma unroll
    for (int k = 0; k < 16; k++) acc[k] = V3{0, 0, 0};
    for (int v = 0; v < V; v++) {
        const V3 cp = {campos[3 * v], campos[3 * v + 1], campos[3 * v + 2]};
        const V3 dir_orig = mean - cp;
        const V3 dir = dir_orig / sqrtf(dot3(dir_orig, dir_orig));
        const float* gp = gcol + ((size_t)v * P + idx) * 3;
        const V3 g = {gp[0], gp[1], gp[2]};
        const float x = dir.x, y = dir.y, z = dir.z;
        V3 t[16];
#pragma unroll
        for (int k = 0; k < 16; k++) t[k] = V3{0, 0, 0};
        t[0] = kSH0 * g;
        if (D > 0) {
            t[1] = (-kSH1 * y) * g;
            t[2] = (kSH1 * z) * g;
            t[3] = (-kSH1 * x) * g;
            if (D > 1) {
                const float xx = x * x, yy = y * y, zz = z * z, xy = x * y, yz = y * z, xz = x * z;
                t[4] = (kSH2[0] * xy) * g;
                t[5] = (kSH2[1] * yz) * g;
                t[6] = (kSH2[2] * (2.f * zz - xx - yy)) * g;
                t[7] = (kSH2[3] * xz) * g;
                t[8] = (kSH2[4] * (xx - yy)) * g;
                if (D > 2) {
                    t[9] = (kSH3[0] * y * (3.f * xx - yy)) * g;
                    t[10] = (kSH3[1] * xy * z) * g;
                    t[11] = (kSH3[2] * y * (4.f * zz - xx - yy)) * g;
                    t[12] = (kSH3[3] * z * (2.f * zz - 3.f * xx - 3.f * yy)) * g;
                    t[13] = (kSH3[4] * x * (4.f * zz - xx - yy)) * g;
                    t[14] = (kSH3[5] * z * (xx - yy)) * g;
                    t[15] = (kSH3[6] * x * (xx - 3.f * yy)) * g;
                }
            }
        }
#pragma unroll
        for (int k = 0; k < 16; k++) acc[k] = v == 0 ? t[k] : acc[k] + t[k];
    }
    float* row = s_dsh + (size_t)threadIdx.x * (3 * M + 1);
#pragma unroll
    for (int k = 0; k < 16; k++)
        if (k < M) {
            row[3 * k] = acc[k].x;
            row[3 * k + 1] = acc[k].y;
            row[3 * k + 2] = acc[k].z;
        }
    __syncthreads();
    const int w = 3 * M;
    const int rows = min(256, P - (int)(blockIdx.x * blockDim.x));
    float* out = dL_dsh + (size_t)blockIdx.x * blockDim.x * w;
    for (int i = threadIdx.x; i < rows * w; i += 256) {
        const int r = i / w, col = i - r * w;
        out[i] = s_dsh[r * (w + 1) + col];
    }
}

__global__ __launch_bounds__(256) void mark_visible_k(int P, const float* __restrict__ means3D, const float* view,
                                                      uint8_t* __restrict__ present) {
    const int idx = blockIdx.x * blockDim.x + threadIdx.x;
    if (idx >= P) return;
    const V3 p = {means3D[3 * idx], means3D[3 * idx + 1], means3D[3 * idx + 2]};
    float m[16];
#pragma unroll
    for (int i = 0; i < 16; i++) m[i] = view[i];
    present[idx] = xform_point_4x3(p, m).z > 0.2f ? 1 : 0;
}

}

void launch_preprocess_fwd(const GoiRasterScene& sc, const GeomView& g, int* radii, uint2* ranges, int n_tiles,
                           hipStream_t s, const float* zcut, uint32_t* zlearn) {
    PreArgs a;
    a.zcut = g_options.cull_variant >= 2 ? zcut : nullptr;
    a.zlearn = zlearn;
    a.P = sc.P; a.D = sc.D; a.M = sc.M; a.W = sc.W; a.H = sc.H;
    a.gx = (sc.W + TILE - 1) / TILE;
    a.gy = (sc.H + TILE - 1) / TILE;
    a.prefiltered = sc.prefiltered;
    a.cull = g_options.cull_variant;
    a.means3D = sc.means3D; a.shs = sc.shs; a.colors_precomp = sc.colors_precomp; a.opacities = sc.opacities;
    a.scales = sc.scales; a.rotations = sc.rotations; a.cov3D_precomp = sc.cov3D_precomp;
    a.scale_modifier = sc.scale_modifier; a.tan_fovx = sc.tan_fovx; a.tan_fovy = sc.tan_fovy;
    a.focal_y = sc.H / (2.0f * sc.tan_fovy);
    a.focal_x = sc.W / (2.0f * sc.tan_fovx);
    a.view_p = sc.viewmatrix; a.proj_p = sc.projmatrix; a.campos_p = sc.campos;
    static_assert(PRE_BLOCK == 256, "preprocess_fwd_k is written for 256-thread workgroups");
    preprocess_fwd_k<<<dim3((sc.P + PRE_BLOCK - 1) / PRE_BLOCK), dim3(PRE_BLOCK), 0, s>>>(
        a, g.rec, g.cov3D, g.tiles_touched, g.clamped, g.sort_keys[1], g.aux, g.blk_agg, g.blk_coarse, radii, g.counters, ranges, n_tiles);
}

void launch_preprocess_bwd(const GoiRasterScene& sc, const GeomView& g, const int* radii, float* dL_dmean2D,
                           const float* dL_dconic, float* dL_dcolor, const float* dL_ddepth, float* dL_dmean3D,
                           float* dL_dcov3D, float* dL_dsh, float* dL_dscale, float* dL_drot, hipStream_t s,
                           const float* record_rows, float* dL_dopacity, float* dL_dsemantic, const int* prev_radii,
                           const uint8_t* row_flags, int N_cap, bool accumulate, int max_blocks) {
    BwdArgs a;
    a.prev_radii = prev_radii;
    a.accumulate = accumulate ? 1 : 0;
    a.P = sc.P; a.D = sc.D; a.M = sc.M; a.W = sc.W; a.H = sc.H;
    a.means3D = sc.means3D; a.shs = sc.shs; a.scales = sc.scales; a.rotations = sc.rotations;
    a.cov3D = sc.cov3D_precomp ? sc.cov3D_precomp : g.cov3D;
    a.scale_modifier = sc.scale_modifier; a.tan_fovx = sc.tan_fovx; a.tan_fovy = sc.tan_fovy;
    a.focal_y = sc.H / (2.0f * sc.tan_fovy);
    a.focal_x = sc.W / (2.0f * sc.tan_fovx);
    a.view_p = sc.viewmatrix; a.proj_p = sc.projmatrix; a.campos_p = sc.campos;
    const bool with_sh = sc.shs && sc.M > 0 && dL_dsh;
    const bool fused = record_rows != nullptr && row_flags != nullptr;
    const int tile_rows = fused ? BWD_TILE_ROWS_FUSED : BWD_TILE_ROWS_DEFAULT;
    const size_t lds = with_sh ? (size_t)tile_rows * (3 * sc.M + 1) * sizeof(float) : 0;
    RecArgs ra;
    ra.rows = record_rows; ra.aux = g.aux; ra.tiles_touched = g.tiles_touched;
    ra.row_floats = bwd_row_floats(sc.S); ra.S = sc.S; ra.nch = 4 * ((sc.S + 3) / 4) + 4;
    ra.dL_dopacity = dL_dopacity; ra.dL_dsemantic = dL_dsemantic;
    ra.flags = row_flags; ra.n_dev = g.counters + COUNTER_N; ra.N_cap = (uint32_t)std::max(N_cap, 0);
    static const int n_cu = []() {
        int dev = 0, n = 256;
        if (hipGetDevice(&dev) == hipSuccess) (void)hipDeviceGetAttribute(&n, hipDeviceAttributeMultiprocessorCount, dev);
        return n > 0 ? n : 256;
    }();
    int blocks = std::min((sc.P + 255) / 256, n_cu * BWD_BLOCKS_PER_CU);
    if (max_blocks > 0) blocks = std::min(blocks, max_blocks);
    const dim3 grid((unsigned)blocks);
#define GOI_PBWD(DSH, SRC, LDS)                                                                                             \
    preprocess_bwd_k<DSH, SRC><<<grid, dim3(256), LDS, s>>>(a, radii, g.counters, g.clamped, dL_dmean2D, dL_dconic, dL_dcolor, \
                                                            dL_ddepth, ra, dL_dmean3D, dL_dcov3D, DSH ? dL_dsh : nullptr,      \
                                                            dL_dscale, dL_drot)
    if (with_sh && fused) GOI_PBWD(true, 2, lds);
    else if (with_sh && record_rows) GOI_PBWD(true, 1, lds);
    else if (with_sh) GOI_PBWD(true, 0, lds);
    else if (fused) GOI_PBWD(false, 2, 0);
    else if (record_rows) GOI_PBWD(false, 1, 0);
    else GOI_PBWD(false, 0, 0);
#undef GOI_PBWD
}

void launch_sh_grad_from_views(int P, int D, int M, int V, const float* means3D, const float* campos, const float* gcol,
                               float* dL_dsh, hipStream_t s) {
    const size_t lds = (size_t)256 * (3 * M + 1) * sizeof(float);
    sh_grad_from_views_k<<<dim3((P + 255) / 256), dim3(256), lds, s>>>(P, D, M, V, means3D, campos, gcol, dL_dsh);
}

void launch_mark_visible(int P, const float* means3D, const float* view, uint8_t* present, hipStream_t s) {
    mark_visible_k<<<dim3((P + 255) / 256), dim3(256), 0, s>>>(P, means3D, view, present);
}

}
```

### goi_hyperplane_amd/csrc/reduce_rows.hip

```cpp
#include <algorithm>
#include <type_traits>

#include "common.h"
#include "row_sum.h"

namespace goi {

namespace {


constexpr uint32_t BIG_INST = REDUCE_BIG_INST;
constexpr uint32_t HUGE_INST = REDUCE_HUGE_INST;

struct ReduceOut {
    float *dL_dmean2D, *dL_dconic, *dL_dopacity, *dL_dcolor, *dL_dsemantic, *dL_ddepth;
};

template <int K, bool RECORD>
__device__ __forceinline__ void store_sums(const float (&sum)[K], float* rows, size_t inst0, uint32_t g, int e, int S, int nch,
                                           const ReduceOut& o) {
    constexpr int RF = 16 * K;
    if constexpr (RECORD) {
        float* dst = rows + inst0 * 4 * RF;
        if (K == 2) {
            reinterpret_cast<float2*>(dst)[e] = make_float2(sum[0], sum[K - 1]);
        } else {
#pragma unroll
            for (int kk = 0; kk < K; kk++) dst[e + 16 * kk] = sum[kk];
        }
    } else {
        const int nsem = nch - 4;
#pragma unroll
        for (int kk = 0; kk < K; kk++) {
            const float v = sum[kk];
            const int el = K == 2 ? 2 * e + kk : e + 16 * kk;
            if (el < nsem) {
                if (el < S) o.dL_dsemantic[(size_t)g * S + el] = v;
            } else if (el < nsem + 3) {
                o.dL_dcolor[(size_t)g * 3 + (el - nsem)] = v;
            } else if (el == nsem + 3) {
                o.dL_ddepth[g] = v;
            } else if (el < nch + 2) {
                o.dL_dmean2D[(size_t)g * 3 + (el - nch)] = v;
                if (el == nch + 1) o.dL_dmean2D[(size_t)g * 3 + 2] = 0.f;
            } else if (el < nch + 5) {
                const int c = el - nch - 2;
                o.dL_dconic[(size_t)g * 4 + (c == 2 ? 3 : c)] = v;
                if (c == 2) o.dL_dconic[(size_t)g * 4 + 2] = 0.f;
            } else if (el == nch + 5) {
                o.dL_dopacity[g] = v;
            }
        }
    }
}

template <int K, int GPQ, bool RECORD, int INFLIGHT = GOI_REDUCE_INFLIGHT>
__global__ __launch_bounds__(256) void reduce_rows_k(int P, int S, int nch, uint32_t N_cap, const uint32_t* __restrict__ n_dev,
                                                     const uint32_t* __restrict__ order,
                                                     const uint32_t* __restrict__ offsets,
                                                     const uint32_t* __restrict__ tiles_touched,
                                                     float* rows, const uint8_t* __restrict__ flags, ReduceOut out,
                                                     uint32_t* __restrict__ big_ctl, uint4* __restrict__ big_desc,
                                                     uint32_t cap_big) {
    const bool truncated = n_dev[COUNTER_OVF - COUNTER_N] != 0;
    const uint32_t N = truncated ? 0u : min(N_cap, *n_dev);
    const int V = truncated ? 0 : (int)n_dev[COUNTER_V - COUNTER_N];
    const int lane = threadIdx.x & 63, quarter = lane >> 4, e = lane & 15;
    const uint32_t* flags32 = reinterpret_cast<const uint32_t*>(flags);
    if constexpr (!RECORD) {
        const int i = blockIdx.x * 256 + threadIdx.x;
        if (i < P && (truncated || tiles_touched[i] == 0)) {
            if ((S & 3) == 0) {
                float4* d4 = reinterpret_cast<float4*>(out.dL_dsemantic + (size_t)i * S);
                for (int ch = 0; ch < S / 4; ch++) d4[ch] = make_float4(0.f, 0.f, 0.f, 0.f);
            } else {
                for (int ch = 0; ch < S; ch++) out.dL_dsemantic[(size_t)i * S + ch] = 0.f;
            }
            if (out.dL_dopacity) {
                out.dL_dopacity[i] = 0.f;
                out.dL_ddepth[i] = 0.f;
#pragma unroll
                for (int k = 0; k < 3; k++) out.dL_dcolor[(size_t)i * 3 + k] = out.dL_dmean2D[(size_t)i * 3 + k] = 0.f;
#pragma unroll
                for (int k = 0; k < 4; k++) out.dL_dconic[(size_t)i * 4 + k] = 0.f;
            }
        }
    }
    const int i0 = blockIdx.x * (16 * GPQ) + (threadIdx.x >> 4);
    if (blockIdx.x * (16 * GPQ) >= V) return;
    struct Meta {
        uint32_t g, off0, off1;
    };
    auto load_meta = [&](int k) {
        const int i = i0 + 16 * k;
        Meta m{0u, 0u, 0u};
        if (k < GPQ && i < V) {
            m.g = order[i];
            m.off0 = min(offsets[i], N);
            m.off1 = i + 1 < V ? min(offsets[i + 1], N) : N;
        }
        return m;
    };
    const uint32_t big_inst = (N > REDUCE_DENSE_RATIO * (uint32_t)V) ? BIG_INST : 1024u;
    auto load_first = [&](const Meta& m) {
        const uint32_t c = m.off1 - m.off0;
        return (c <= big_inst && (uint32_t)e < c) ? flags32[m.off0 + e] : 0u;
    };

    Meta cur = load_meta(0), nxt = load_meta(1);
    uint32_t w_cur = load_first(cur);
#pragma unroll 1
    for (int k = 0; k < GPQ; k++) {
        if (i0 + 16 * k - (int)(threadIdx.x >> 4) >= V) break;
        const Meta nn = load_meta(k + 2);
        const uint32_t w_nxt = load_first(nxt);
        const bool live = i0 + 16 * k < V;
        const uint32_t cnt_all = cur.off1 - cur.off0;
        const bool big = cnt_all > big_inst;
        const size_t inst0 = cur.off0;
        if (big && e == 0) {
            const uint4 d = make_uint4((uint32_t)inst0, cnt_all, 0u, cur.g);
            if (cnt_all > HUGE_INST) big_desc[atomicAdd(&big_ctl[1], 1u)] = d;
            else big_desc[cap_big - 1u - atomicAdd(&big_ctl[2], 1u)] = d;
        }
        const uint32_t cnt = big ? 0u : cnt_all;
        float sum[K];
#pragma unroll
        for (int kk = 0; kk < K; kk++) sum[kk] = 0.f;
        sum_instances<K, false, INFLIGHT>(rows, flags32, inst0, cnt, w_cur, quarter, e, sum, sum);
        if (live && !big && (!RECORD || cnt > 0)) store_sums<K, RECORD>(sum, rows, inst0, cur.g, e, S, nch, out);
        cur = nxt;
        nxt = nn;
        w_cur = w_nxt;
    }
}

__global__ __launch_bounds__(256) void find_big_k(uint32_t N_cap, const uint32_t* __restrict__ n_dev,
                                                  const uint32_t* __restrict__ order, const uint32_t* __restrict__ offsets,
                                                  uint32_t* __restrict__ big_ctl, uint4* __restrict__ big_desc, uint32_t cap_big) {
    const bool truncated = n_dev[COUNTER_OVF - COUNTER_N] != 0;
    const uint32_t N = truncated ? 0u : min(N_cap, *n_dev);
    const int V = truncated ? 0 : (int)n_dev[COUNTER_V - COUNTER_N];
    const int i = blockIdx.x * 256 + threadIdx.x;
    if (i >= V) return;
    const uint32_t off0 = min(offsets[i], N), off1 = i + 1 < V ? min(offsets[i + 1], N) : N;
    const uint32_t cnt = off1 - off0;
    const uint32_t big_inst = (N > REDUCE_DENSE_RATIO * (uint32_t)V) ? BIG_INST : 1024u;
    if (cnt > big_inst) {
        const uint4 d = make_uint4(off0, cnt, 0u, order[i]);
        if (cnt > HUGE_INST) big_desc[atomicAdd(&big_ctl[1], 1u)] = d;
        else big_desc[cap_big - 1u - atomicAdd(&big_ctl[2], 1u)] = d;
    }
}

constexpr int BIG_PARTS = 64, MID_PARTS = 16;
template <int K, bool RECORD>
__global__ __launch_bounds__(16 * BIG_PARTS) void reduce_big_k(const uint32_t* __restrict__ big_ctl,
                                                              const uint4* __restrict__ big_desc, uint32_t cap_big, float* rows,
                                                              const uint8_t* __restrict__ flags, int S, int nch, ReduceOut out) {
    constexpr int RF = 16 * K;
    __shared__ float s_part[BIG_PARTS][RF];
    const int lane = threadIdx.x & 63, quarter = lane >> 4, e = lane & 15, part = threadIdx.x >> 4;
    const uint32_t* flags32 = reinterpret_cast<const uint32_t*>(flags);
    auto one = [&](const uint4 d, bool active, int parts, int first) {
        const int p = part - first;
        const uint32_t n = active ? d.y : 0u;
        const uint32_t per = ((n + (uint32_t)parts - 1u) / (uint32_t)parts + 63u) & ~63u;
        const uint32_t p0 = min(n, (uint32_t)p * per), p1 = min(n, (uint32_t)(p + 1) * per);
        const uint32_t cnt = p1 - p0;
        const size_t inst0 = (size_t)d.x + p0;
        const uint32_t w0 = ((uint32_t)e < cnt) ? flags32[inst0 + e] : 0u;
        float sum[K], comp[K];
#pragma unroll
        for (int kk = 0; kk < K; kk++) sum[kk] = comp[kk] = 0.f;
        sum_instances<K, true>(rows, flags32, inst0, cnt, w0, quarter, e, sum, comp);
#pragma unroll
        for (int kk = 0; kk < K; kk++) s_part[part][K == 2 ? 2 * e + kk : e + 16 * kk] = sum[kk];
        __syncthreads();
        if (p == 0 && active) {
            float tot[K], c[K];
#pragma unroll
            for (int kk = 0; kk < K; kk++) tot[kk] = c[kk] = 0.f;
            for (int pp = 0; pp < parts; pp++)
#pragma unroll
                for (int kk = 0; kk < K; kk++) {
                    const float y = s_part[first + pp][K == 2 ? 2 * e + kk : e + 16 * kk] - c[kk];
                    const float t = tot[kk] + y;
                    c[kk] = (t - tot[kk]) - y;
                    tot[kk] = t;
                }
            store_sums<K, RECORD>(tot, rows, (size_t)d.x, d.w, e, S, nch, out);
        }
        __syncthreads();
    };
    const uint32_t nmid = big_ctl[2], nhuge = big_ctl[1];
    const int sub = part / MID_PARTS;
    for (uint32_t b0 = blockIdx.x * 4u; b0 < nmid; b0 += gridDim.x * 4u) {
        const uint32_t b = b0 + (uint32_t)sub;
        const bool active = b < nmid;
        const uint4 d = active ? big_desc[cap_big - 1u - b] : make_uint4(0u, 0u, 0u, 0u);
        one(d, active, MID_PARTS, sub * MID_PARTS);
    }
    for (uint32_t b = blockIdx.x; b < nhuge; b += gridDim.x) one(big_desc[b], true, BIG_PARTS, 0);
}

}

#ifndef GOI_REDUCE_GPQ
#define GOI_REDUCE_GPQ 2
#endif
constexpr int REDUCE_GPQ = GOI_REDUCE_GPQ;
#ifndef GOI_REDUCE_BIG_GRID
#define GOI_REDUCE_BIG_GRID 512
#endif
constexpr size_t REDUCE_BIG_GRID = GOI_REDUCE_BIG_GRID;

#ifndef GOI_REDUCE_LARGE_SCENE
#define GOI_REDUCE_LARGE_SCENE 2000000
#endif
constexpr int REDUCE_LARGE_SCENE = GOI_REDUCE_LARGE_SCENE;
template <int K, bool RECORD>
static void launch_reduce_k(const GoiRasterScene& sc, const GeomView& g, int N, int nch, float* rows, const uint8_t* flags,
                            const BwdScratchView& scr, const ReduceOut& out, hipStream_t s) {
    const dim3 grid((sc.P + 16 * REDUCE_GPQ - 1) / (16 * REDUCE_GPQ));
    const uint32_t* order = g.sort_vals[depth_sort_result_index()];
    if (sc.P >= REDUCE_LARGE_SCENE && GOI_REDUCE_INFLIGHT > 16)
        reduce_rows_k<K, 1, RECORD, 16><<<dim3((sc.P + 15) / 16), dim3(256), 0, s>>>(sc.P, sc.S, nch, (uint32_t)N, g.counters + COUNTER_N,
                                                                                    order, g.offsets, g.tiles_touched, rows, flags, out,
                                                                                    scr.big_ctl, scr.big_desc, (uint32_t)scr.cap_big);
    else
        reduce_rows_k<K, REDUCE_GPQ, RECORD><<<grid, dim3(256), 0, s>>>(sc.P, sc.S, nch, (uint32_t)N, g.counters + COUNTER_N, order,
                                                                        g.offsets, g.tiles_touched, rows, flags, out, scr.big_ctl,
                                                                        scr.big_desc, (uint32_t)scr.cap_big);
    if (N > 0)
        reduce_big_k<K, RECORD><<<dim3((unsigned)std::min<size_t>(REDUCE_BIG_GRID, scr.cap_big)), dim3(16 * BIG_PARTS), 0, s>>>(
            scr.big_ctl, scr.big_desc, (uint32_t)scr.cap_big, rows, flags, sc.S, nch, out);
}

void launch_reduce_rows(const GoiRasterScene& sc, const GeomView& g, int N, const BwdScratchView& scr, float* dL_dmean2D,
                        float* dL_dconic, float* dL_dopacity, float* dL_dcolor, float* dL_dsemantic, float* dL_ddepth,
                        hipStream_t s, bool records) {
    const int rf = bwd_row_floats(sc.S), nch = 4 * ((sc.S + 3) / 4) + 4;
    const ReduceOut out{dL_dmean2D, dL_dconic, dL_dopacity, dL_dcolor, dL_dsemantic, dL_ddepth};
#define GOI_REDUCE(K)                                                                   \
    do {                                                                                \
        if (records) launch_reduce_k<K, true>(sc, g, N, nch, scr.rows, scr.flags, scr, out, s);  \
        else launch_reduce_k<K, false>(sc, g, N, nch, scr.rows, scr.flags, scr, out, s);         \
    } while (0)
    if (rf == 32) GOI_REDUCE(2);
    else if (rf == 16) GOI_REDUCE(1);
    else GOI_REDUCE(3);
#undef GOI_REDUCE
}

void launch_reduce_big_only(const GoiRasterScene& sc, const GeomView& g, int N, const BwdScratchView& scr, hipStream_t s) {
    if (N <= 0) return;
    const int nch = 4 * ((sc.S + 3) / 4) + 4;
    const ReduceOut out{nullptr, nullptr, nullptr, nullptr, nullptr, nullptr};
    const uint32_t* order = g.sort_vals[depth_sort_result_index()];
    find_big_k<<<dim3((sc.P + 255) / 256), dim3(256), 0, s>>>((uint32_t)N, g.counters + COUNTER_N, order, g.offsets, scr.big_ctl,
                                                             scr.big_desc, (uint32_t)scr.cap_big);
    reduce_big_k<2, true><<<dim3((unsigned)std::min<size_t>(REDUCE_BIG_GRID, scr.cap_big)), dim3(16 * BIG_PARTS), 0, s>>>(
        scr.big_ctl, scr.big_desc, (uint32_t)scr.cap_big, scr.rows, scr.flags, sc.S, nch, out);
}

void launch_reduce_sem_rows(const GoiRasterScene& sc, const GeomView& g, int N, const BwdScratchView& scr, int row_floats,
                            float* dL_dsemantic, hipStream_t s) {
    const int nch = row_floats + 4;
    const ReduceOut out{nullptr, nullptr, nullptr, nullptr, dL_dsemantic, nullptr};
    if (row_floats == 16) launch_reduce_k<1, false>(sc, g, N, nch, scr.rows, scr.flags, scr, out, s);
    else launch_reduce_k<2, false>(sc, g, N, nch, scr.rows, scr.flags, scr, out, s);
}

}
```

### goi_hyperplane_amd/csrc/row_sum.h

```cpp
#pragma once
#include "common.h"

namespace goi {

#ifndef GOI_REDUCE_INFLIGHT
#define GOI_REDUCE_INFLIGHT 32
#endif

template <int K, bool COMPENSATED = false, int INFLIGHT = GOI_REDUCE_INFLIGHT>
__device__ __forceinline__ void sum_instances(const float* __restrict__ rows, const uint32_t* __restrict__ flags32,
                                              size_t inst0, uint32_t cnt, uint32_t w_first, int quarter, int e,
                                              float (&sum)[K], float (&comp)[K]) {
    constexpr int RF = 16 * K;
    auto load_flags = [&](uint32_t c) { return (c + e < cnt) ? flags32[inst0 + c + e] : 0u; };
    uint32_t cmax = cnt;
#pragma unroll
    for (int d = 32; d >= 16; d >>= 1) cmax = max(cmax, (uint32_t)__shfl_xor((int)cmax, d, 64));
    uint32_t wq[4] = {w_first, 0u, 0u, 0u};
    if (cmax > 16) {
#pragma unroll
        for (int sblk = 1; sblk < 4; sblk++) wq[sblk] = load_flags(16u * sblk);
    }
    for (uint32_t c = 0; c < cmax; c += 64) {
        uint32_t wn[4] = {0u, 0u, 0u, 0u};
        if (c + 64 < cmax) {
#pragma unroll
            for (int sblk = 0; sblk < 4; sblk++) wn[sblk] = load_flags(c + 64 + 16u * sblk);
        }
#pragma unroll 1
        for (int sblk = 0; sblk < 4; sblk++) {
            const uint32_t cc = c + 16u * sblk;
            if (cc >= cmax) break;
            const uint32_t w = wq[0];
            wq[0] = wq[1];
            wq[1] = wq[2];
            wq[2] = wq[3];
            if (__ballot(w != 0u) == 0) continue;
            unsigned long long m = 0;
#pragma unroll
            for (int q = 0; q < 4; q++) {
                const unsigned long long bal = __ballot(((w >> (8 * q)) & 0xFFu) != 0);
                m |= ((bal >> (16 * quarter)) & 0xFFFFull) << (16 * q);
            }
            const float* chunk = rows + (inst0 + cc) * 4 * RF;
            auto trip = [&](auto nf_c) {
                constexpr int NF = decltype(nf_c)::value;
                float v[NF][K];
#pragma unroll
                for (int i = 0; i < NF; i++) {
                    const bool have = m != 0;
                    const int bit = have ? __builtin_ctzll(m) : 0;
                    if (have) m &= m - 1;
                    const float* r = chunk + (size_t)((bit & 15) * 4 + (bit >> 4)) * RF;
                    if (K == 2) {
                        const float2 t = have ? reinterpret_cast<const float2*>(r)[e] : make_float2(0.f, 0.f);
                        v[i][0] = t.x;
                        v[i][K - 1] = t.y;
                    } else {
#pragma unroll
                        for (int kk = 0; kk < K; kk++) v[i][kk] = have ? r[e + 16 * kk] : 0.f;
                    }
                }
#pragma unroll
                for (int i = 0; i < NF; i++)
#pragma unroll
                    for (int kk = 0; kk < K; kk++) {
                        if constexpr (COMPENSATED) {
                            const float y = v[i][kk] - comp[kk];
                            const float t = sum[kk] + y;
                            comp[kk] = (t - sum[kk]) - y;
                            sum[kk] = t;
                        } else {
                            sum[kk] += v[i][kk];
                        }
                    }
            };
            int left = __popcll(m);
#pragma unroll
            for (int d = 32; d >= 16; d >>= 1) left = max(left, __shfl_xor(left, d, 64));
            left = __builtin_amdgcn_readfirstlane(left);
            while (left > 0) {
                if (left <= 4) {
                    trip(std::integral_constant<int, 4>{});
                    left -= 4;
                } else if (left <= 12) {
                    trip(std::integral_constant<int, 12>{});
                    left -= 12;
                } else {
                    trip(std::integral_constant<int, INFLIGHT>{});
                    left -= INFLIGHT;
                }
            }
        }
#pragma unroll
        for (int sblk = 0; sblk < 4; sblk++) wq[sblk] = wn[sblk];
    }
}

}
```

### goi_hyperplane_amd/csrc/torch_binding.cpp

```cpp
#include <torch/extension.h>

#include <c10/hip/HIPGuard.h>
#include <c10/hip/HIPStream.h>

#include <cstdlib>
#include <map>
#include <mutex>
#include <tuple>
#include <vector>

#include "goi_raster.h"

namespace {

using torch::Tensor;

void* grow(void* user, size_t bytes) {
    auto* t = static_cast<Tensor*>(user);
    const long long step = 16ll << 20;
    t->resize_({((long long)bytes + step - 1) / step * step});
    return t->data_ptr();
}

struct Arg {
// ... 96 lines not shown
    f.a[5] = arg(opacity, "opacities", dev);
    f.a[6] = arg(scales, "scales", dev);
    f.a[7] = arg(rotations, "rotations", dev);
    f.a[8] = arg(cov3D_precomp, "cov3D_precomp", dev);
    f.a[9] = arg(viewmatrix, "viewmatrix", dev);
    f.a[10] = arg(projmatrix, "projmatrix", dev);
    f.a[11] = arg(campos, "campos", dev);
    f.sc = scene_of(f.P, degree, sh, f.S, f.W, f.H, f.a[0], f.a[1], f.a[2], f.a[3], f.a[4], f.a[5], f.a[6], scale_modifier,
                    f.a[7], f.a[8], f.a[9], f.a[10], f.a[11], tan_fovx, tan_fovy, prefiltered, debug);
    return f;
}

std::tuple<int, Tensor, Tensor, Tensor, Tensor, Tensor, Tensor, Tensor, Tensor> rasterize_gaussians(GOI_FORWARD_ARGS) {
    Prepared f = prepare(background, means3D, colors, semantics, opacity, scales, rotations, scale_modifier, cov3D_precomp,
                         viewmatrix, projmatrix, tan_fovx, tan_fovy, image_height, image_width, sh, degree, campos,
                         prefiltered, debug, true);
    c10::hip::HIPGuard guard(f.dev.index());
    auto f32 = means3D.options().dtype(torch::kFloat32);
    auto bytes = means3D.options().dtype(torch::kByte);
    Tensor out_color = torch::empty({3, f.H, f.W}, f32), out_sem = torch::empty({f.S, f.H, f.W}, f32);
    Tensor out_depth = torch::empty({1, f.H, f.W}, f32), out_alpha = torch::empty({1, f.H, f.W}, f32);
    Tensor radii = torch::empty({f.P}, means3D.options().dtype(torch::kInt32));
    Tensor geom = torch::empty({f.P > 0 ? (long long)goi_raster_geom_bytes(f.P) : 0}, bytes);
    Tensor img = torch::empty({f.P > 0 ? (long long)goi_raster_image_bytes(f.W, f.H) : 0}, bytes);
    Tensor binning = torch::empty({0}, bytes);
    const int n = goi_raster_forward(&f.sc, f.P ? geom.data_ptr() : nullptr, f.P ? img.data_ptr() : nullptr, grow, &binning,
                                     out_color.data_ptr<float>(), out_sem.data_ptr<float>(), out_depth.data_ptr<float>(),
                                     out_alpha.data_ptr<float>(), f.P ? radii.data_ptr<int>() : nullptr, stream_of(f.dev));
    if (n < 0) raise_last();
    return std::make_tuple(n, out_color, out_sem, out_depth, out_alpha, radii, geom, binning, img);
}

std::tuple<int, Tensor, Tensor, Tensor, Tensor, Tensor, Tensor, Tensor, Tensor> rasterize_gaussians_async(
    GOI_FORWARD_ARGS, const int capacity, const c10::optional<Tensor>& zcut_in, const c10::optional<Tensor>& zcut_out) {
    Prepared f = prepare(background, means3D, colors, semantics, opacity, scales, rotations, scale_modifier, cov3D_precomp,
                         viewmatrix, projmatrix, tan_fovx, tan_fovy, image_height, image_width, sh, degree, campos,
                         prefiltered, debug, true);
    c10::hip::HIPGuard guard(f.dev.index());
    auto f32 = means3D.options().dtype(torch::kFloat32);
    auto bytes = means3D.options().dtype(torch::kByte);
    Tensor out_color = torch::empty({3, f.H, f.W}, f32), out_sem = torch::empty({f.S, f.H, f.W}, f32);
    Tensor out_depth = torch::empty({1, f.H, f.W}, f32), out_alpha = torch::empty({1, f.H, f.W}, f32);
    Tensor radii = torch::empty({f.P}, means3D.options().dtype(torch::kInt32));
    Tensor geom = torch::empty({(long long)goi_raster_geom_bytes(f.P)}, bytes);
    Tensor img = torch::empty({(long long)goi_raster_image_bytes(f.W, f.H)}, bytes);
    const long long step = 16ll << 20;
    Tensor binning = torch::empty({((long long)goi_raster_binning_bytes(capacity) + step - 1) / step * step}, bytes);
    const long long tiles = ((long long)(f.W + 15) / 16) * ((f.H + 15) / 16);
    const float* zin = nullptr;
    float* zout = nullptr;
    for (int k = 0; k < 2; k++) {
        const auto& z = k == 0 ? zcut_in : zcut_out;
        if (!z.has_value() || !z->defined()) continue;
        TORCH_CHECK(z->scalar_type() == torch::kFloat32 && z->is_contiguous() && z->device() == f.dev && z->numel() == tiles,
                    "zcut arrays must be contiguous float32 [tiles] tensors on the frame's device");
        if (k == 0) zin = z->data_ptr<float>();
        else zout = z->data_ptr<float>();
    }
    const int ticket = goi_raster_forward_async_cut(&f.sc, geom.data_ptr(), img.data_ptr(), binning.data_ptr(), capacity,
                                                    out_color.data_ptr<float>(), out_sem.data_ptr<float>(),
                                                    out_depth.data_ptr<float>(), out_alpha.data_ptr<float>(),
                                                    radii.data_ptr<int>(), zin, zout, stream_of(f.dev));
    if (ticket < 0) raise_last();
    return std::make_tuple(ticket, out_color, out_sem, out_depth, out_alpha, radii, geom, binning, img);
}

std::mutex g_scratch_mu;
std::map<std::pair<int, void*>, Tensor>& g_scratch = *new std::map<std::pair<int, void*>, Tensor>;

void* backward_scratch(size_t bytes, const c10::Device& dev, void* stream, const torch::TensorOptions& byte_opts) {
    std::lock_guard<std::mutex> lk(g_scratch_mu);
    auto key = std::make_pair((int)dev.index(), stream);
    auto it = g_scratch.find(key);
    if (it == g_scratch.end() || (size_t)it->second.numel() < bytes) {
        if (it != g_scratch.end()) g_scratch.erase(it);
        g_scratch[key] = torch::empty({(long long)(bytes + bytes / 4) + 256}, byte_opts);
        it = g_scratch.find(key);
    }
    return it->second.data_ptr();
}

struct PoolEntry {
    Tensor all;
    Tensor prev_radii;
    int64_t version;
};
struct PoolKey {
    int dev;
    void* stream;
    long long total;
    int P, M, S;
    bool operator<(const PoolKey& o) const {
        return std::tie(dev, stream, total, P, M, S) < std::tie(o.dev, o.stream, o.total, o.P, o.M, o.S);
    }
};
std::mutex g_pool_mu;
std::map<PoolKey, std::vector<PoolEntry>>& g_pool = *new std::map<PoolKey, std::vector<PoolEntry>>;
bool g_pool_on = []() {
    const char* e = std::getenv("GOI_GRAD_POOL");
    return !(e && (e[0] == '0' || e[0] == 'n' || e[0] == 'f'));
}();
long long g_pool_hits = 0, g_pool_dirty = 0, g_pool_fresh = 0;
constexpr size_t POOL_BUFFERS_PER_KEY = 3;

void set_grad_pool(bool on) {
    std::lock_guard<std::mutex> lk(g_pool_mu);
    g_pool_on = on;
    if (!on) g_pool.clear();
}
std::tuple<long long, long long, long long> grad_pool_stats() {
    std::lock_guard<std::mutex> lk(g_pool_mu);
    return std::make_tuple(g_pool_hits, g_pool_dirty, g_pool_fresh);
}

long long release_scratch() {
    long long freed = 0;
    {
        std::lock_guard<std::mutex> lk(g_scratch_mu);
        for (auto& kv : g_scratch) freed += kv.second.numel();
        g_scratch.clear();
    }
    std::lock_guard<std::mutex> lk(g_pool_mu);
    for (auto& kv : g_pool)
        for (auto& e : kv.second) freed += e.all.numel() * 4;
    g_pool.clear();
    return freed;
}

std::tuple<Tensor, Tensor, Tensor, Tensor, Tensor, Tensor, Tensor, Tensor, Tensor> backward_ex(
    const Tensor& background, const Tensor& means3D, const Tensor& radii, const Tensor& colors, const Tensor& semantics,
    const Tensor& scales, const Tensor& rotations, const float scale_modifier, const Tensor& cov3D_precomp,
    const Tensor& viewmatrix, const Tensor& projmatrix, const float tan_fovx, const float tan_fovy,
    const c10::optional<Tensor>& dL_dout_color, const c10::optional<Tensor>& dL_dout_semantic,
    const c10::optional<Tensor>& dL_dout_depth, const c10::optional<Tensor>& dL_dout_alpha, const Tensor& sh,
    const int degree, const Tensor& campos, const Tensor& geomBuffer, const int R, const Tensor& binningBuffer,
    const Tensor& imageBuffer, const Tensor& alphas, const bool debug, const bool sh_factored_in,
    const int scratch_instances ,
    const c10::optional<Tensor>& accumulate_into ) {
    const c10::Device dev = check_device(means3D);
    c10::hip::HIPGuard guard(dev.index());
    const int P = (int)means3D.size(0);
    const int H = (int)alphas.size(-2), W = (int)alphas.size(-1);
    const int S = (int)semantics.size(1);
    const int M = (sh.defined() && sh.numel()) ? (int)sh.size(1) : 0;
    const bool sh_factored = sh_factored_in && M > 0;
    auto f32 = means3D.options().dtype(torch::kFloat32);
    const long long sizes[11] = {3ll * P, sh_factored ? 0ll : 3ll * M * P, (long long)S * P, (long long)P, 3ll * P, 4ll * P,
                                 3ll * P, 3ll * P, (long long)P, 4ll * P, 6ll * P};
    long long offs[11], total = 0;
    for (int i = 0; i < 11; i++) {
        offs[i] = total;
        total += (sizes[i] + 63) / 64 * 64;
    }
    void* stream = stream_of(dev);
    Tensor flat, prev_radii;
    const PoolKey key{(int)dev.index(), stream, total, P, sh_factored ? -M : M, S};
    const bool accumulate = accumulate_into.has_value() && accumulate_into->defined() && P != 0;
    if (accumulate) {
        const Tensor& first = *accumulate_into;
        TORCH_CHECK(!sh_factored, "accumulate_into: not with the factored dL/dSH");
        TORCH_CHECK(first.is_cuda() && first.device() == dev && first.scalar_type() == torch::kFloat32 && first.storage_offset() == 0 &&
                        (long long)(first.storage().nbytes() / sizeof(float)) >= total,
                    "accumulate_into must be the dL_dmeans3D an earlier backward of the same shapes returned");
        flat = torch::empty({0}, f32).set_(first.storage(), 0, {total}, {1});
        first.unsafeGetTensorImpl()->bump_version();
    } else if (P != 0) {
        std::lock_guard<std::mutex> lk(g_pool_mu);
        if (g_pool_on) {
            auto& v = g_pool[key];
            for (size_t i = 0; i < v.size(); i++) {
                if (v[i].all.storage().use_count() != 1 || v[i].all.use_count() != 1) continue;
                flat = v[i].all;
                if ((int64_t)flat._version() == v[i].version) {
                    prev_radii = v[i].prev_radii;
                    g_pool_hits++;
                } else {
                    g_pool_dirty++;
                }
                v.erase(v.begin() + i);
                break;
            }
        }
    }
    if (!flat.defined()) {
        flat = torch::empty({total}, f32);
        g_pool_fresh++;
    }
    auto view = [&](int i, at::IntArrayRef shape) { return flat.narrow(0, offs[i], sizes[i]).view(shape); };
    Tensor dL_dmeans3D = view(0, {P, 3});
    Tensor dL_dsh = sh_factored ? Tensor() : view(1, {P, M, 3});
    Tensor dL_dsemantics = view(2, {P, S});
    Tensor dL_dopacity = view(3, {P, 1});
    Tensor dL_dscales = view(4, {P, 3});
    Tensor dL_drotations = view(5, {P, 4});
    Tensor dL_dmeans2D = view(6, {P, 3}), dL_dcolors = view(7, {P, 3});
    Tensor dL_ddepths = view(8, {P, 1}), dL_dconic = view(9, {P, 2, 2});
    Tensor dL_dcov3D = view(10, {P, 6});
    if (P != 0) {
        Arg bg = arg(background, "background", dev), m3 = arg(means3D, "means3D", dev), shs = arg(sh, "sh", dev);
        Arg col = arg(colors, "colors_precomp", dev), sem = arg(semantics, "semantics", dev);
        Arg sca = arg(scales, "scales", dev), rot = arg(rotations, "rotations", dev);
        Arg cov = arg(cov3D_precomp, "cov3D_precomp", dev), vm = arg(viewmatrix, "viewmatrix", dev);
        Arg pm = arg(projmatrix, "projmatrix", dev), cp = arg(campos, "campos", dev), al = arg(alphas, "alphas", dev);
        Arg gc = arg(dL_dout_color, "dL_dout_color", dev), gs = arg(dL_dout_semantic, "dL_dout_semantic", dev);
        Arg gd = arg(dL_dout_depth, "dL_dout_depth", dev), ga = arg(dL_dout_alpha, "dL_dout_alpha", dev);
        TORCH_CHECK_TYPE(radii.scalar_type() == torch::kInt32, "radii must be torch.int32");
        Tensor rad = radii.contiguous();
        GoiRasterScene sc = scene_of(P, degree, sh, S, W, H, bg, m3, shs, col, sem, Arg(), sca, scale_modifier, rot, cov, vm,
                                     pm, cp, tan_fovx, tan_fovy, false, debug);
        void* scratch = backward_scratch(goi_raster_backward_scratch_bytes(scratch_instances > 0 ? scratch_instances : R, S), dev,
                                         stream, means3D.options().dtype(torch::kByte));
        const int r = goi_raster_backward3(
            &sc, R, scratch_instances, accumulate ? GOI_BACKWARD_ACCUMULATE : 0, geomBuffer.data_ptr(), binningBuffer.numel() ? binningBuffer.data_ptr() : nullptr,
            imageBuffer.data_ptr(), rad.data_ptr<int>(), al.p, gc.p, gs.p, gd.p, ga.p, dL_dmeans2D.data_ptr<float>(),
            dL_dconic.data_ptr<float>(), dL_dopacity.data_ptr<float>(), dL_dcolors.data_ptr<float>(),
            dL_dsemantics.data_ptr<float>(), dL_ddepths.data_ptr<float>(), dL_dmeans3D.data_ptr<float>(),
            dL_dcov3D.data_ptr<float>(), dL_dsh.defined() && dL_dsh.numel() ? dL_dsh.data_ptr<float>() : nullptr,
            dL_dscales.data_ptr<float>(), dL_drotations.data_ptr<float>(), scratch,
            prev_radii.defined() ? prev_radii.data_ptr<int>() : nullptr, stream);
        if (r < 0) raise_last();
        std::lock_guard<std::mutex> lk(g_pool_mu);
        if (g_pool_on && !debug && !accumulate) {
            auto& v = g_pool[key];
            if (v.size() >= POOL_BUFFERS_PER_KEY) v.erase(v.begin());
            v.push_back(PoolEntry{flat, rad, (int64_t)flat._version()});
        }
    }
    flat = Tensor();
    return std::make_tuple(dL_dmeans2D, dL_dcolors, dL_dsemantics, dL_dopacity, dL_dmeans3D, dL_dcov3D, dL_dsh,
                           dL_dscales, dL_drotations);
}

std::tuple<Tensor, Tensor, Tensor, Tensor, Tensor, Tensor, Tensor, Tensor, Tensor> rasterize_gaussians_backward(
    const Tensor& background, const Tensor& means3D, const Tensor& radii, const Tensor& colors, const Tensor& semantics,
    const Tensor& scales, const Tensor& rotations, const float scale_modifier, const Tensor& cov3D_precomp,
    const Tensor& viewmatrix, const Tensor& projmatrix, const float tan_fovx, const float tan_fovy,
    const Tensor& dL_dout_color, const Tensor& dL_dout_semantic, const Tensor& dL_dout_depth, const Tensor& dL_dout_alpha,
    const Tensor& sh, const int degree, const Tensor& campos, const Tensor& geomBuffer, const int R,
    const Tensor& binningBuffer, const Tensor& imageBuffer, const Tensor& alphas, const bool debug) {
    return backward_ex(background, means3D, radii, colors, semantics, scales, rotations, scale_modifier, cov3D_precomp,
                       viewmatrix, projmatrix, tan_fovx, tan_fovy, dL_dout_color, dL_dout_semantic, dL_dout_depth,
                       dL_dout_alpha, sh, degree, campos, geomBuffer, R, binningBuffer, imageBuffer, alphas, debug, false, 0, c10::nullopt);
}

Tensor backward_semantics(const Tensor& background, const Tensor& means3D, const Tensor& radii, const Tensor& semantics,
                          const Tensor& viewmatrix, const Tensor& projmatrix, const float tan_fovx, const float tan_fovy,
                          const Tensor& dL_dout_semantic, const Tensor& campos, const Tensor& geomBuffer, const int R,
                          const Tensor& binningBuffer, const Tensor& imageBuffer, const Tensor& alphas, const int sh_degree,
                          const bool debug) {
    const c10::Device dev = check_device(means3D);
    c10::hip::HIPGuard guard(dev.index());
    const int P = (int)means3D.size(0), S = (int)dL_dout_semantic.size(0);
    const int H = (int)dL_dout_semantic.size(1), W = (int)dL_dout_semantic.size(2);
    Tensor dL_dsemantics = torch::empty({P, S}, means3D.options().dtype(torch::kFloat32));
    if (P != 0) {
        Arg bg = arg(background, "background", dev), m3 = arg(means3D, "means3D", dev), sem = arg(semantics, "semantics", dev);
        Arg vm = arg(viewmatrix, "viewmatrix", dev), pm = arg(projmatrix, "projmatrix", dev), cp = arg(campos, "campos", dev);
        Arg al = arg(alphas, "alphas", dev), gs = arg(dL_dout_semantic, "dL_dout_semantic", dev);
        Tensor rad = radii.contiguous();
        GoiRasterScene sc = scene_of(P, sh_degree, Tensor(), S, W, H, bg, m3, Arg(), m3, sem, Arg(), Arg(), 1.0f, Arg(), m3, vm,
                                     pm, cp, tan_fovx, tan_fovy, false, debug);
        void* stream = stream_of(dev);
        void* scratch = backward_scratch(goi_raster_backward_scratch_bytes(R, S), dev, stream,
                                         means3D.options().dtype(torch::kByte));
        if (goi_raster_backward_semantics(&sc, R, geomBuffer.data_ptr(),
                                          binningBuffer.numel() ? binningBuffer.data_ptr() : nullptr,
                                          imageBuffer.data_ptr(), rad.data_ptr<int>(), al.p, gs.p,
                                          dL_dsemantics.data_ptr<float>(), scratch, stream) < 0)
            raise_last();
    }
    return dL_dsemantics;
}

std::tuple<int, Tensor, Tensor, Tensor, Tensor, Tensor, Tensor> rasterize_gaussians_trace(
    const Tensor& background, const Tensor& means3D, const Tensor& colors, const Tensor& img_sem, const Tensor& opacity,
    const Tensor& scales, const Tensor& rotations, const float scale_modifier, const Tensor& cov3D_precomp,
    const Tensor& viewmatrix, const Tensor& projmatrix, const float tan_fovx, const float tan_fovy, const int image_height,
    const int image_width, const Tensor& sh, const int degree, const Tensor& campos, const bool prefiltered,
    const bool debug) {
    TORCH_CHECK(img_sem.defined() && img_sem.numel() > 0, "img_sem [S,H,W] is required");
    Prepared f = prepare(background, means3D, colors, img_sem, opacity, scales, rotations, scale_modifier, cov3D_precomp,
                         viewmatrix, projmatrix, tan_fovx, tan_fovy, image_height, image_width, sh, degree, campos,
                         prefiltered, debug, false);
    c10::hip::HIPGuard guard(f.dev.index());
    Arg img_in = arg(img_sem, "img_sem", f.dev);
    auto f32 = means3D.options().dtype(torch::kFloat32);
    auto bytes = means3D.options().dtype(torch::kByte);
    Tensor out_color = torch::empty({3, f.H, f.W}, f32);
    Tensor gau_sem = torch::zeros({f.P, f.S}, f32);
    Tensor num_gsem = torch::zeros({f.P}, means3D.options().dtype(torch::kInt32));
    Tensor radii = torch::empty({f.P}, means3D.options().dtype(torch::kInt32));
    Tensor geom = torch::empty({f.P > 0 ? (long long)goi_raster_geom_bytes(f.P) : 0}, bytes);
    Tensor img = torch::empty({f.P > 0 ? (long long)goi_raster_image_bytes(f.W, f.H) : 0}, bytes);
    Tensor binning = torch::empty({0}, bytes);
    const int n = goi_raster_trace(&f.sc, img_in.p, f.P ? geom.data_ptr() : nullptr, f.P ? img.data_ptr() : nullptr, grow,
                                   &binning, out_color.data_ptr<float>(), f.P ? gau_sem.data_ptr<float>() : nullptr,
                                   f.P ? num_gsem.data_ptr<int>() : nullptr, f.P ? radii.data_ptr<int>() : nullptr,
                                   stream_of(f.dev));
    if (n < 0) raise_last();
    return std::make_tuple(n, out_color, gau_sem, num_gsem, geom, binning, img);
}

Tensor mark_visible(const Tensor& means3D, const Tensor& viewmatrix, const Tensor& projmatrix) {
    const c10::Device dev = check_device(means3D);
    c10::hip::HIPGuard guard(dev.index());
    const int P = (int)means3D.size(0);
    Tensor present = torch::zeros({P}, means3D.options().dtype(torch::kBool));
    if (P != 0) {
// ... 31 lines not shown
```

### include/goi_raster.h

```cpp
#ifndef GOI_RASTER_H
#define GOI_RASTER_H

#include <stddef.h>
#include <stdint.h>

#ifdef __cplusplus
extern "C" {
#endif

#define GOI_RASTER_ABI_VERSION 6

typedef struct GoiRasterScene {
    int P;
    int D;
    int M;
    int S;
    int W, H;
    const float* bg;
    const float* means3D;
    const float* shs;
    const float* colors_precomp;
    const float* semantics;
    const float* opacities;
    const float* scales;
    float scale_modifier;
    const float* rotations;
    const float* cov3D_precomp;
    const float* viewmatrix;
    const float* projmatrix;
    const float* campos;
    float tan_fovx, tan_fovy;
    int prefiltered;
    int debug;
} GoiRasterScene;

typedef void* (*goi_alloc_fn)(void* user, size_t bytes);

int goi_raster_abi_version(void);
const char* goi_raster_last_error(void);

size_t goi_raster_geom_bytes(int P);
size_t goi_raster_image_bytes(int W, int H);
size_t goi_raster_binning_bytes(int num_rendered);
size_t goi_raster_backward_scratch_bytes(int num_rendered, int S);

int goi_raster_forward(const GoiRasterScene* scene, void* geom_buffer, void* image_buffer,
                       goi_alloc_fn binning_alloc, void* alloc_user,
                       float* out_color, float* out_semantic, float* out_depth, float* out_alpha,
                       int* radii, void* stream);

int goi_raster_forward_async(const GoiRasterScene* scene, void* geom_buffer, void* image_buffer, void* binning_buffer,
                             int capacity, float* out_color, float* out_semantic, float* out_depth, float* out_alpha,
                             int* radii, void* stream);
int goi_raster_ticket_result(int ticket, int wait, int* num_rendered);

int goi_raster_forward_async_cut(const GoiRasterScene* scene, void* geom_buffer, void* image_buffer, void* binning_buffer,
                                 int capacity, float* out_color, float* out_semantic, float* out_depth, float* out_alpha,
                                 int* radii, const float* zcut_in, float* zcut_out, void* stream);
int goi_raster_ticket_result2(int ticket, int wait, int* num_rendered, unsigned* frame_flags);
#define GOI_FRAME_TRUNCATED 1u
#define GOI_FRAME_MISSORTED 2u
#define GOI_FRAME_CUT_TOO_TIGHT 4u
const uint32_t* goi_raster_truncated_flag(const void* geom_buffer, int P);
int goi_raster_forward_redo(const GoiRasterScene* scene, int num_rendered, void* geom_buffer, void* image_buffer,
                            void* binning_buffer, float* out_color, float* out_semantic, float* out_depth,
                            float* out_alpha, const int* radii, void* stream);

int goi_raster_forward_reblend(const GoiRasterScene* scene, int R, const void* geom_buffer, const void* binning_buffer,
                               const void* cached_image_buffer, void* image_buffer, float* out_color, float* out_semantic,
                               float* out_depth, float* out_alpha, void* stream);

int goi_raster_backward(const GoiRasterScene* scene, int R,
                        const void* geom_buffer, const void* binning_buffer, const void* image_buffer,
                        const int* radii, const float* out_alpha,
                        const float* dL_dout_color, const float* dL_dout_semantic,
                        const float* dL_dout_depth, const float* dL_dout_alpha,
                        float* dL_dmean2D , float* dL_dconic , float* dL_dopacity ,
                        float* dL_dcolor , float* dL_dsemantic , float* dL_ddepth ,
                        float* dL_dmean3D , float* dL_dcov3D , float* dL_dsh ,
                        float* dL_dscale , float* dL_drot ,
                        void* scratch ,
                        void* stream);

int goi_raster_backward2(const GoiRasterScene* scene, int R, const void* geom_buffer, const void* binning_buffer,
                         const void* image_buffer, const int* radii, const float* out_alpha, const float* dL_dout_color,
                         const float* dL_dout_semantic, const float* dL_dout_depth, const float* dL_dout_alpha,
                         float* dL_dmean2D, float* dL_dconic, float* dL_dopacity, float* dL_dcolor, float* dL_dsemantic,
                         float* dL_ddepth, float* dL_dmean3D, float* dL_dcov3D, float* dL_dsh, float* dL_dscale,
                         float* dL_drot, void* scratch, const int* prev_radii, void* stream);

#define GOI_BACKWARD_ACCUMULATE 1
int goi_raster_backward3(const GoiRasterScene* scene, int R, int scratch_instances, int flags, const void* geom_buffer,
                         const void* binning_buffer, const void* image_buffer, const int* radii, const float* out_alpha,
                         const float* dL_dout_color, const float* dL_dout_semantic, const float* dL_dout_depth,
                         const float* dL_dout_alpha, float* dL_dmean2D, float* dL_dconic, float* dL_dopacity, float* dL_dcolor,
                         float* dL_dsemantic, float* dL_ddepth, float* dL_dmean3D, float* dL_dcov3D, float* dL_dsh,
                         float* dL_dscale, float* dL_drot, void* scratch, const int* prev_radii, void* stream);

int goi_raster_backward_semantics(const GoiRasterScene* scene, int R, const void* geom_buffer,
                                  const void* binning_buffer, const void* image_buffer, const int* radii,
                                  const float* out_alpha, const float* dL_dout_semantic, float* dL_dsemantic,
                                  void* scratch, void* stream);

int goi_raster_trace(const GoiRasterScene* scene, const float* img_sem, void* geom_buffer, void* image_buffer,
                     goi_alloc_fn binning_alloc, void* alloc_user,
                     float* out_color, float* gau_sem, int* num_gsem, int* radii, void* stream);

int goi_raster_mark_visible(int P, const float* means3D, const float* viewmatrix, const float* projmatrix,
                            uint8_t* present, void* stream);

int goi_semantic_decode(const float* sem, int S, long long HW, const float* W, const float* bias, int n_codes,
                        const float* code_score, float thresh, float* sim_out, int* idx_out, uint8_t* bg_mask_out,
                        void* stream);

#define GOI_OSH_MAX_EPOCHS 1000000
int goi_semantic_osh_counts(const int* idx, const uint8_t* positive, long long HW, int n_codes, int* counts, void* stream);
int goi_semantic_osh_fit(const float* lut, int n_codes, int D, const int* counts, long long HW, int K, float* w, float* b,
                         float lr, int max_epochs, double target_iou, int* epochs_out, float* loss_out, double* iou_out,
                         double* init_iou_out, double* trace, void* stream);

#define DBSCAN_FLAG_NONFINITE 1
#define DBSCAN_FLAG_SORT 2
#define DBSCAN_FLAG_RANGE 4
#define DBSCAN_FLAG_GRID 8
#define DBSCAN_FLAG_UNION 16
size_t goi_semantic_dbscan_workspace_bytes(long long n);
int goi_semantic_dbscan(long long n, const float* points, float eps, int min_samples, int* labels, uint8_t* core, int* result,
                        void* workspace, void* stream);

#define GOI_MASK_F32 0
#define GOI_MASK_U8 1
#define GOI_MASK_MAX_RADIUS 63
int goi_semantic_mask_pack(const void* src, int src_dtype, int n_views, int H, int W, int first_view, uint64_t* packed, long long* counts,
                  void* stream);
int goi_semantic_mask_dilate(const uint64_t* src, uint64_t* dst, int n_views, int H, int W, int radius, void* stream);
int goi_semantic_mask_unpack(const uint64_t* packed, int n_views, int H, int W, int n_out, const long long* index, uint8_t* out,
                             void* stream);
int goi_semantic_mask_confusion(const uint64_t* pred, const uint64_t* gt, int n_views, int H, int W, long long* out, void* stream);

#define GOI_CODEBOOK_FLAG_NONFINITE 1
#define GOI_CODEBOOK_FLAG_SORT 2
#define GOI_CODEBOOK_FLAG_TABLE 4
#define GOI_CODEBOOK_RANK_MAX 4096
#define GOI_CODEBOOK_KMEANS_MAX_K 4096
#define GOI_CODEBOOK_KMEANS_MAX_DIM 1024
size_t goi_codebook_unique_rows_workspace_bytes(int n_views, int D, int H, int W);
int goi_codebook_unique_rows(const float* const* maps, int n_views, int D, int H, int W, long long* counts, unsigned* flags,
                             goi_alloc_fn alloc, void* alloc_user, void* workspace, void* stream);
size_t goi_codebook_kmeans_workspace_bytes(long long n_rows, int n_problems, int ncluster, int D);
int goi_codebook_kmeans(float* x, const long long* row_offsets, int n_problems, long long max_rows, long long n_rows, int D,
                        int ncluster, int niter, const int* perms, float* centers, int* status, void* workspace, void* stream);

#define GOI_PHOTOMETRIC_WINDOW 11
#define GOI_PHOTOMETRIC_GRAD1 1u
#define GOI_PHOTOMETRIC_GRAD2 2u
#define GOI_PHOTOMETRIC_PER_IMAGE 4u
#define GOI_PHOTOMETRIC_SSIM_ONLY 8u
size_t goi_raster_photometric_workspace_bytes(long long n, int c, int h, int w, unsigned flags);
int goi_raster_photometric_forward(const float* img1, const float* img2, long long n, int c, int h, int w, int window_size,
                                   float lambda_dssim, unsigned flags, float* out, float* out_images, void* workspace, void* stream);
int goi_raster_photometric_backward(const float* img1, const float* img2, long long n, int c, int h, int w, int window_size,
                                    float lambda_dssim, unsigned flags, const float* grad_out, const void* workspace, float* grad1,
                                    float* grad2, void* stream);

enum {
    GOI_STAGE_PREPROCESS = 0,
    GOI_STAGE_DEPTH_SORT,
    GOI_STAGE_SCAN,
    GOI_STAGE_EMIT,
    GOI_STAGE_TILE_SORT,
    GOI_STAGE_RANGES,
    GOI_STAGE_BLEND_FWD,
    GOI_STAGE_BLEND_BWD,
    GOI_STAGE_PREPROCESS_BWD,
    GOI_STAGE_COUNT
};
void goi_raster_profile_enable(int on);
void goi_raster_profile_stages(unsigned stage_mask);
int goi_raster_profile_collect(double* ms, int* calls);

int goi_raster_set_option(const char* name, int value);
// ... 113 lines not shown
```

Measured before the change: 755.2.

## Skip backward preprocess for visible Gaussians with no blend contribution

The row reduction now records a per-Gaussian contribution byte telling whether any pixel produced a nonzero gradient row. The preprocess-backward kernel uses that byte instead of mere visibility to decide which Gaussians get the full chain-rule work, and it zeroes or keeps the rest. A per-Gaussian row mask is written and pooled so the next call knows which gradient slots are already zero, replacing the prev_radii tensor. The kernel also prefetches the next segment's radii and flags. This adds scratch space and a byte read per Gaussian, and correctness depends on the contrib flags and the pooled mask staying consistent.

New measurement: 801.6 (median of 6 runs). 6.2% higher.

```diff
diff --git a/goi_hyperplane_amd/_C.py b/goi_hyperplane_amd/_C.py
--- a/goi_hyperplane_amd/_C.py
+++ b/goi_hyperplane_amd/_C.py
@@ -862,12 +862,12 @@
                 binningBuffer = lazy_binning
             R_scratch = _scratch_instances(R, R_layout)
             scratch = _backward_scratch(lib.goi_raster_backward_scratch_bytes(R_scratch or R_layout, S), dev)
-            r = lib.goi_raster_backward3(
+            r = lib.goi_raster_backward4(
                 C.byref(sc), R_layout, R_scratch, 0, _ptr(geomBuffer), _ptr(binningBuffer), _ptr(imageBuffer), _ptr(ten["radii"]),
                 _ptr(ten["alphas"]), _ptr(ten["g_c"]), _ptr(ten["g_s"]), _ptr(ten["g_d"]), _ptr(ten["g_a"]),
                 _ptr(dL_dmeans2D), _ptr(dL_dconic), _ptr(dL_dopacity), _ptr(dL_dcolors), _ptr(dL_dsemantics),
                 _ptr(dL_ddepths), _ptr(dL_dmeans3D), _ptr(dL_dcov3D), _ptr(dL_dsh), _ptr(dL_dscales),
-                _ptr(dL_drotations), _ptr(scratch), None, _stream(dev))
+                _ptr(dL_drotations), _ptr(scratch), None, None, None, _stream(dev))
             if r < 0:
                 raise RuntimeError(_lib.last_error())
     return (dL_dmeans2D, dL_dcolors, dL_dsemantics, dL_dopacity, dL_dmeans3D, dL_dcov3D, dL_dsh, dL_dscales,
diff --git a/goi_hyperplane_amd/_lib.py b/goi_hyperplane_amd/_lib.py
--- a/goi_hyperplane_amd/_lib.py
+++ b/goi_hyperplane_amd/_lib.py
@@ -6,7 +6,7 @@
 _HERE = os.path.dirname(os.path.abspath(__file__))
 LIB_PATH = os.path.join(_HERE, "lib", "libgoi_raster.so")
 
-ABI_VERSION = 6
+ABI_VERSION = 7
 
 STAGES = ("preprocess", "depth_sort", "scan", "emit", "tile_sort", "ranges", "blend_fwd", "blend_bwd",
           "preprocess_bwd")
@@ -49,6 +49,9 @@
                              + [C.c_void_p] * 11 + [C.c_void_p, C.c_void_p, C.c_void_p]),
     "goi_raster_backward3": (C.c_int, [C.POINTER(GoiRasterScene), C.c_int, C.c_int, C.c_int] + [C.c_void_p] * 3 + [C.c_void_p] * 6
                              + [C.c_void_p] * 11 + [C.c_void_p, C.c_void_p, C.c_void_p]),
+    "goi_raster_backward4": (C.c_int, [C.POINTER(GoiRasterScene), C.c_int, C.c_int, C.c_int] + [C.c_void_p] * 3 + [C.c_void_p] * 6
+                             + [C.c_void_p] * 11 + [C.c_void_p, C.c_void_p, C.c_void_p, C.c_void_p, C.c_void_p]),
+    "goi_raster_debug_backward_contrib_offset": (C.c_size_t, [C.c_int, C.c_int]),
     "goi_raster_backward_semantics": (C.c_int, [C.POINTER(GoiRasterScene), C.c_int] + [C.c_void_p] * 9),
     "goi_raster_trace": (C.c_int, [C.POINTER(GoiRasterScene), C.c_void_p, C.c_void_p, C.c_void_p, ALLOC_FN,
                                    C.c_void_p] + [C.c_void_p] * 4 + [C.c_void_p]),
diff --git a/goi_hyperplane_amd/csrc/api.hip b/goi_hyperplane_amd/csrc/api.hip
--- a/goi_hyperplane_amd/csrc/api.hip
+++ b/goi_hyperplane_amd/csrc/api.hip
@@ -401,6 +401,7 @@
     b.cap_big = reduce_cap_big(n / 4);
     carve(p, b.big_ctl, 8);
     carve(p, b.big_desc, b.cap_big);
+    carve(p, b.contrib, n / 4);
     return (size_t)(p - base) + 256;
 }
 
@@ -432,6 +433,11 @@
 size_t goi_raster_image_bytes(int W, int H) { return image_layout(W, H, nullptr, nullptr) + 256; }
 size_t goi_raster_binning_bytes(int N) { return binning_layout(N, nullptr, nullptr) + 256; }
 size_t goi_raster_backward_scratch_bytes(int N, int S) { return bwd_scratch_layout(N, S, nullptr, nullptr) + 256; }
+size_t goi_raster_debug_backward_contrib_offset(int N, int S) {
+    BwdScratchView v;
+    bwd_scratch_layout(N, S, nullptr, &v);
+    return reinterpret_cast<size_t>(v.contrib);
+}
 
 int goi_raster_forward(const GoiRasterScene* scene, void* geom_buffer, void* image_buffer, goi_alloc_fn binning_alloc,
                        void* alloc_user, float* out_color, float* out_semantic, float* out_depth, float* out_alpha,
@@ -651,6 +657,19 @@
                          const float* dL_dout_alpha, float* dL_dmean2D, float* dL_dconic, float* dL_dopacity, float* dL_dcolor,
                          float* dL_dsemantic, float* dL_ddepth, float* dL_dmean3D, float* dL_dcov3D, float* dL_dsh,
                          float* dL_dscale, float* dL_drot, void* scratch, const int* prev_radii, void* stream) {
+    return goi_raster_backward4(scene, R, scratch_instances, flags, geom_buffer, binning_buffer, image_buffer, radii, out_alpha,
+                                dL_dout_color, dL_dout_semantic, dL_dout_depth, dL_dout_alpha, dL_dmean2D, dL_dconic, dL_dopacity,
+                                dL_dcolor, dL_dsemantic, dL_ddepth, dL_dmean3D, dL_dcov3D, dL_dsh, dL_dscale, dL_drot, scratch,
+                                prev_radii, nullptr, nullptr, stream);
+}
+
+int goi_raster_backward4(const GoiRasterScene* scene, int R, int scratch_instances, int flags, const void* geom_buffer,
+                         const void* binning_buffer, const void* image_buffer, const int* radii, const float* out_alpha,
+                         const float* dL_dout_color, const float* dL_dout_semantic, const float* dL_dout_depth,
+                         const float* dL_dout_alpha, float* dL_dmean2D, float* dL_dconic, float* dL_dopacity, float* dL_dcolor,
+                         float* dL_dsemantic, float* dL_ddepth, float* dL_dmean3D, float* dL_dcov3D, float* dL_dsh,
+                         float* dL_dscale, float* dL_drot, void* scratch, const int* prev_radii, const uint8_t* prev_mask,
+                         uint8_t* row_mask, void* stream) {
     refresh_options();
     if (validate(scene, true, false)) return -1;
     const GoiRasterScene& sc = *scene;
@@ -672,6 +691,7 @@
     if (accumulate && (!rows_path || g_options.bwd_records != 1 || prev_radii || (sc.shs && !dL_dsh) || sc.debug))
         return fail("GOI_BACKWARD_ACCUMULATE needs the default backward (scratch given, bwd_variant 0 / 2, bwd_records 1), dL_dsh when "
                     "the colours are SH, prev_radii NULL and debug off");
+    if (accumulate && (prev_mask || row_mask)) return fail("GOI_BACKWARD_ACCUMULATE: prev_mask and row_mask must be NULL");
     if (rows_path) {
         BwdScratchView scr;
         bwd_scratch_layout(Rs, sc.S, static_cast<char*>(scratch), &scr);
@@ -691,15 +711,19 @@
         if (g_options.bwd_records == 2 && bwd_row_floats(sc.S) == 32 && R > 0 && !accumulate) {
             launch_reduce_big_only(sc, g, Rs, scr, s);
             launch_preprocess_bwd(sc, g, radii, dL_dmean2D, dL_dconic, dL_dcolor, dL_ddepth, dL_dmean3D, dL_dcov3D, dL_dsh,
-                                  dL_dscale, dL_drot, s, scr.rows, dL_dopacity, dL_dsemantic, prev_radii, scr.flags, Rs);
+                                  dL_dscale, dL_drot, s, scr.rows, dL_dopacity, dL_dsemantic, prev_radii, scr.flags, Rs, false, 0,
+                                  nullptr, prev_mask, row_mask);
         } else if (g_options.bwd_records) {
-            launch_reduce_rows(sc, g, Rs, scr, nullptr, nullptr, nullptr, nullptr, nullptr, nullptr, s, true);
+            uint8_t* contrib = g_options.bwd_skip_idle ? scr.contrib : nullptr;
+            launch_reduce_rows(sc, g, Rs, scr, nullptr, nullptr, nullptr, nullptr, nullptr, nullptr, s, true, contrib);
             launch_preprocess_bwd(sc, g, radii, dL_dmean2D, dL_dconic, dL_dcolor, dL_ddepth, dL_dmean3D, dL_dcov3D, dL_dsh,
-                                  dL_dscale, dL_drot, s, scr.rows, dL_dopacity, dL_dsemantic, prev_radii, nullptr, 0, accumulate);
+                                  dL_dscale, dL_drot, s, scr.rows, dL_dopacity, dL_dsemantic, prev_radii, nullptr, 0, accumulate, 0,
+                                  contrib, prev_mask, row_mask);
         } else {
             launch_reduce_rows(sc, g, Rs, scr, dL_dmean2D, dL_dconic, dL_dopacity, dL_dcolor, dL_dsemantic, dL_ddepth, s);
             launch_preprocess_bwd(sc, g, radii, dL_dmean2D, dL_dconic, dL_dcolor, dL_ddepth, dL_dmean3D, dL_dcov3D, dL_dsh,
-                                  dL_dscale, dL_drot, s);
+                                  dL_dscale, dL_drot, s, nullptr, nullptr, nullptr, nullptr, nullptr, 0, false, 0, nullptr, nullptr,
+                                  row_mask);
         }
     } else {
         GOI_HIP(hipMemsetAsync(dL_dmean2D, 0, 3 * P * sizeof(float), s));
@@ -717,7 +741,8 @@
         if (check_stage(sc, s, "backward blend")) return -1;
         StageTimer t(GOI_STAGE_PREPROCESS_BWD, s);
         launch_preprocess_bwd(sc, g, radii, dL_dmean2D, dL_dconic, dL_dcolor, dL_ddepth, dL_dmean3D, dL_dcov3D, dL_dsh,
-                              dL_dscale, dL_drot, s);
+                              dL_dscale, dL_drot, s, nullptr, nullptr, nullptr, nullptr, nullptr, 0, false, 0, nullptr, nullptr,
+                              row_mask);
     }
     if (check_stage(sc, s, "backward preprocess")) return -1;
     GOI_HIP(hipGetLastError());
@@ -1237,6 +1262,10 @@
     else if (!strcmp(name, "bwd_records")) {
         if (value < 0 || value > 2) return fail("bwd_records must be 0, 1 or 2");
         g_options.bwd_records = value;
+    }
+    else if (!strcmp(name, "bwd_skip_idle")) {
+        if (value < 0 || value > 1) return fail("bwd_skip_idle must be 0 or 1");
+        g_options.bwd_skip_idle = value;
     }
     else if (!strcmp(name, "osh_path")) {
         if (value < 0 || value > 1) return fail("osh_path must be 0 or 1");
diff --git a/goi_hyperplane_amd/csrc/common.h b/goi_hyperplane_amd/csrc/common.h
--- a/goi_hyperplane_amd/csrc/common.h
+++ b/goi_hyperplane_amd/csrc/common.h
@@ -59,6 +59,7 @@
     uint32_t* big_ctl;
     uint4* big_desc;
     size_t cap_big;
+    uint8_t* contrib;
 };
 size_t bwd_scratch_layout(int N, int S, char* base, BwdScratchView* v);
 
@@ -90,6 +91,7 @@
     int bwd_order = 1;
     int bwd_masks = 1;
     int bwd_records = 1;
+    int bwd_skip_idle = 1;
     int osh_path = 0;
 };
 extern thread_local Options g_options;
@@ -147,7 +149,8 @@
                             float* dL_dsemantic, hipStream_t s);
 void launch_reduce_rows(const GoiRasterScene& sc, const GeomView& g, int N, const BwdScratchView& scr, float* dL_dmean2D,
                         float* dL_dconic, float* dL_dopacity, float* dL_dcolor, float* dL_dsemantic, float* dL_ddepth,
-                        hipStream_t s, bool records = false);
+                        hipStream_t s, bool records = false,
+                        uint8_t* contrib = nullptr);
 void launch_render_bwd_tile(const GoiRasterScene& sc, const GeomView& g, const ImageView& im,
                             const uint32_t* point_list, const float* out_alpha, const float* dL_dpix,
                             const float* dL_dsem, const float* dL_ddepth, const float* dL_dalpha, float* dL_dmean2D,
@@ -162,7 +165,9 @@
                            const int* prev_radii = nullptr,
                            const uint8_t* row_flags = nullptr, int N_cap = 0,
                            bool accumulate = false,
-                           int max_blocks = 0);
+                           int max_blocks = 0,
+                           const uint8_t* contrib = nullptr,
+                           const uint8_t* prev_mask = nullptr, uint8_t* row_mask = nullptr);
 int launch_semantic_decode(const float* sem, int S, long long HW, const float* W, const float* bias, int n_codes,
                            const float* code_score, float thresh, float* sim_out, int* idx_out, uint8_t* bg_mask_out,
                            hipStream_t s);
diff --git a/goi_hyperplane_amd/csrc/preprocess.hip b/goi_hyperplane_amd/csrc/preprocess.hip
--- a/goi_hyperplane_amd/csrc/preprocess.hip
+++ b/goi_hyperplane_amd/csrc/preprocess.hip
@@ -334,6 +334,8 @@
     const float* proj_p;
     const float* campos_p;
     const int* prev_radii;
+    const uint8_t* prev_mask;
+    uint8_t* row_mask;
     int accumulate;
 };
 
@@ -347,6 +349,7 @@
     const uint8_t* flags;
     const uint32_t* n_dev;
     uint32_t N_cap;
+    const uint8_t* contrib;
 };
 #ifndef GOI_PBWD_ROWS
 #define GOI_PBWD_ROWS 224
@@ -400,17 +403,43 @@
     const int nseg = (args.P + 255) / 256;
     const bool truncated = counters[COUNTER_OVF] != 0;
     int npend = 0;
+    const bool skip_idle = SRC == 1 && ra.contrib != nullptr;
+    struct SegIn {
+        int rad;
+        uint32_t tt, ax;
+        uint32_t prev;
+    };
+    auto load_seg = [&](int sg) {
+        SegIn v{0, 0u, 0u, 1u};
+        const int id = sg * 256 + (int)threadIdx.x;
+        if (sg < nseg && id < args.P) {
+            v.rad = radii[id];
+            if (skip_idle) {
+                v.tt = ra.tiles_touched[id];
+                v.ax = ra.aux[id].x;
+            }
+            if (args.prev_mask != nullptr) v.prev = args.prev_mask[id];
+            else if (args.prev_radii != nullptr) v.prev = args.prev_radii[id] != 0 ? 1u : 0u;
+        }
+        return v;
+    };
+    SegIn cur = load_seg(blockIdx.x);
     for (int seg = blockIdx.x; seg < nseg || npend > 0; seg += gridDim.x) {
     int nzero = 0;
     const int base = seg * 256;
+    const bool vis_t = cur.rad > 0 && !truncated;
+    const bool listed_t = skip_idle && vis_t && cur.tt != 0u;
+    const uint8_t contrib_t = listed_t ? ra.contrib[cur.ax] : (uint8_t)0;
+    const SegIn nxt = load_seg(seg + (int)gridDim.x);
     if (seg < nseg) {
         const int gtid = base + threadIdx.x;
         const bool live = gtid < args.P;
-        const bool vis_t = live && radii[gtid] > 0 && !truncated;
-        const bool keep_t = live && !vis_t && args.prev_radii != nullptr && args.prev_radii[gtid] == 0;
-        const bool zero_t = live && !vis_t && !keep_t && !args.accumulate;
+        const bool work_t = skip_idle ? contrib_t != 0 : vis_t;
+        const bool keep_t = live && !work_t && cur.prev == 0u;
+        const bool zero_t = live && !work_t && !keep_t && !args.accumulate;
+        if (args.row_mask != nullptr && live) args.row_mask[gtid] = work_t ? (uint8_t)1 : (uint8_t)0;
         const int wv = threadIdx.x >> 6;
-        const unsigned long long bv = __ballot(vis_t), bz = __ballot(zero_t);
+        const unsigned long long bv = __ballot(work_t), bz = __ballot(zero_t);
         if ((threadIdx.x & 63) == 0) {
             s_wcnt[0][wv] = __popcll(bv);
             s_wcnt[1][wv] = __popcll(bz);
@@ -424,7 +453,7 @@
         const int nv = s_wcnt[0][0] + s_wcnt[0][1] + s_wcnt[0][2] + s_wcnt[0][3];
         nzero = s_wcnt[1][0] + s_wcnt[1][1] + s_wcnt[1][2] + s_wcnt[1][3];
         const unsigned long long lt = (1ull << (threadIdx.x & 63)) - 1ull;
-        if (vis_t) s_vis[npend + ov + __popcll(bv & lt)] = (uint32_t)gtid;
+        if (work_t) s_vis[npend + ov + __popcll(bv & lt)] = (uint32_t)gtid;
         if (zero_t) s_zero[oz + __popcll(bz & lt)] = (uint16_t)threadIdx.x;
         npend += nv;
         __syncthreads();
@@ -896,6 +925,7 @@
     npend = rest;
     __syncthreads();
     }
+    cur = nxt;
     }
 }
 
@@ -1002,9 +1032,12 @@
                            const float* dL_dconic, float* dL_dcolor, const float* dL_ddepth, float* dL_dmean3D,
                            float* dL_dcov3D, float* dL_dsh, float* dL_dscale, float* dL_drot, hipStream_t s,
                            const float* record_rows, float* dL_dopacity, float* dL_dsemantic, const int* prev_radii,
-                           const uint8_t* row_flags, int N_cap, bool accumulate, int max_blocks) {
+                           const uint8_t* row_flags, int N_cap, bool accumulate, int max_blocks, const uint8_t* contrib,
+                           const uint8_t* prev_mask, uint8_t* row_mask) {
     BwdArgs a;
     a.prev_radii = prev_radii;
+    a.prev_mask = prev_mask;
+    a.row_mask = row_mask;
     a.accumulate = accumulate ? 1 : 0;
     a.P = sc.P; a.D = sc.D; a.M = sc.M; a.W = sc.W; a.H = sc.H;
     a.means3D = sc.means3D; a.shs = sc.shs; a.scales = sc.scales; a.rotations = sc.rotations;
@@ -1022,6 +1055,7 @@
     ra.row_floats = bwd_row_floats(sc.S); ra.S = sc.S; ra.nch = 4 * ((sc.S + 3) / 4) + 4;
     ra.dL_dopacity = dL_dopacity; ra.dL_dsemantic = dL_dsemantic;
     ra.flags = row_flags; ra.n_dev = g.counters + COUNTER_N; ra.N_cap = (uint32_t)std::max(N_cap, 0);
+    ra.contrib = (record_rows != nullptr && !fused) ? contrib : nullptr;
     static const int n_cu = []() {
         int dev = 0, n = 256;
         if (hipGetDevice(&dev) == hipSuccess) (void)hipDeviceGetAttribute(&n, hipDeviceAttributeMultiprocessorCount, dev);
diff --git a/goi_hyperplane_amd/csrc/reduce_rows.hip b/goi_hyperplane_amd/csrc/reduce_rows.hip
--- a/goi_hyperplane_amd/csrc/reduce_rows.hip
+++ b/goi_hyperplane_amd/csrc/reduce_rows.hip
@@ -61,7 +61,7 @@
                                                      const uint32_t* __restrict__ tiles_touched,
                                                      float* rows, const uint8_t* __restrict__ flags, ReduceOut out,
                                                      uint32_t* __restrict__ big_ctl, uint4* __restrict__ big_desc,
-                                                     uint32_t cap_big) {
+                                                     uint32_t cap_big, uint8_t* __restrict__ contrib) {
     const bool truncated = n_dev[COUNTER_OVF - COUNTER_N] != 0;
     const uint32_t N = truncated ? 0u : min(N_cap, *n_dev);
     const int V = truncated ? 0 : (int)n_dev[COUNTER_V - COUNTER_N];
@@ -127,8 +127,15 @@
         float sum[K];
 #pragma unroll
         for (int kk = 0; kk < K; kk++) sum[kk] = 0.f;
-        sum_instances<K, false, INFLIGHT>(rows, flags32, inst0, cnt, w_cur, quarter, e, sum, sum);
-        if (live && !big && (!RECORD || cnt > 0)) store_sums<K, RECORD>(sum, rows, inst0, cur.g, e, S, nch, out);
+        const bool any = sum_instances<K, false, INFLIGHT>(rows, flags32, inst0, cnt, w_cur, quarter, e, sum, sum);
+        if constexpr (RECORD) {
+            if (live && !big && cnt > 0) {
+                if (contrib && e == 0) contrib[inst0] = any ? (uint8_t)1 : (uint8_t)0;
+                if (any || !contrib) store_sums<K, RECORD>(sum, rows, inst0, cur.g, e, S, nch, out);
+            }
+        } else {
+            if (live && !big) store_sums<K, RECORD>(sum, rows, inst0, cur.g, e, S, nch, out);
+        }
         cur = nxt;
         nxt = nn;
         w_cur = w_nxt;
@@ -157,9 +164,11 @@
 template <int K, bool RECORD>
 __global__ __launch_bounds__(16 * BIG_PARTS) void reduce_big_k(const uint32_t* __restrict__ big_ctl,
                                                               const uint4* __restrict__ big_desc, uint32_t cap_big, float* rows,
-                                                              const uint8_t* __restrict__ flags, int S, int nch, ReduceOut out) {
+                                                              const uint8_t* __restrict__ flags, int S, int nch, ReduceOut out,
+                                                              uint8_t* __restrict__ contrib) {
     constexpr int RF = 16 * K;
     __shared__ float s_part[BIG_PARTS][RF];
+    __shared__ uint8_t s_any[BIG_PARTS];
     const int lane = threadIdx.x & 63, quarter = lane >> 4, e = lane & 15, part = threadIdx.x >> 4;
     const uint32_t* flags32 = reinterpret_cast<const uint32_t*>(flags);
     auto one = [&](const uint4 d, bool active, int parts, int first) {
@@ -173,9 +182,10 @@
         float sum[K], comp[K];
 #pragma unroll
         for (int kk = 0; kk < K; kk++) sum[kk] = comp[kk] = 0.f;
-        sum_instances<K, true>(rows, flags32, inst0, cnt, w0, quarter, e, sum, comp);
+        const bool any = sum_instances<K, true>(rows, flags32, inst0, cnt, w0, quarter, e, sum, comp);
 #pragma unroll
         for (int kk = 0; kk < K; kk++) s_part[part][K == 2 ? 2 * e + kk : e + 16 * kk] = sum[kk];
+        if (e == 0) s_any[part] = any ? (uint8_t)1 : (uint8_t)0;
         __syncthreads();
         if (p == 0 && active) {
             float tot[K], c[K];
@@ -190,6 +200,13 @@
                     tot[kk] = t;
                 }
             store_sums<K, RECORD>(tot, rows, (size_t)d.x, d.w, e, S, nch, out);
+            if constexpr (RECORD) {
+                if (contrib && e == 0) {
+                    uint8_t a = 0;
+                    for (int pp = 0; pp < parts; pp++) a |= s_any[first + pp];
+                    contrib[d.x] = a;
+                }
+            }
         }
         __syncthreads();
     };
@@ -221,30 +238,30 @@
 constexpr int REDUCE_LARGE_SCENE = GOI_REDUCE_LARGE_SCENE;
 template <int K, bool RECORD>
 static void launch_reduce_k(const GoiRasterScene& sc, const GeomView& g, int N, int nch, float* rows, const uint8_t* flags,
-                            const BwdScratchView& scr, const ReduceOut& out, hipStream_t s) {
+                            const BwdScratchView& scr, const ReduceOut& out, hipStream_t s, uint8_t* contrib = nullptr) {
     const dim3 grid((sc.P + 16 * REDUCE_GPQ - 1) / (16 * REDUCE_GPQ));
     const uint32_t* order = g.sort_vals[depth_sort_result_index()];
     if (sc.P >= REDUCE_LARGE_SCENE && GOI_REDUCE_INFLIGHT > 16)
         reduce_rows_k<K, 1, RECORD, 16><<<dim3((sc.P + 15) / 16), dim3(256), 0, s>>>(sc.P, sc.S, nch, (uint32_t)N, g.counters + COUNTER_N,
                                                                                     order, g.offsets, g.tiles_touched, rows, flags, out,
-                                                                                    scr.big_ctl, scr.big_desc, (uint32_t)scr.cap_big);
+                                                                                    scr.big_ctl, scr.big_desc, (uint32_t)scr.cap_big, contrib);
     else
         reduce_rows_k<K, REDUCE_GPQ, RECORD><<<grid, dim3(256), 0, s>>>(sc.P, sc.S, nch, (uint32_t)N, g.counters + COUNTER_N, order,
                                                                         g.offsets, g.tiles_touched, rows, flags, out, scr.big_ctl,
-                                                                        scr.big_desc, (uint32_t)scr.cap_big);
+                                                                        scr.big_desc, (uint32_t)scr.cap_big, contrib);
     if (N > 0)
         reduce_big_k<K, RECORD><<<dim3((unsigned)std::min<size_t>(REDUCE_BIG_GRID, scr.cap_big)), dim3(16 * BIG_PARTS), 0, s>>>(
-            scr.big_ctl, scr.big_desc, (uint32_t)scr.cap_big, rows, flags, sc.S, nch, out);
+            scr.big_ctl, scr.big_desc, (uint32_t)scr.cap_big, rows, flags, sc.S, nch, out, contrib);
 }
 
 void launch_reduce_rows(const GoiRasterScene& sc, const GeomView& g, int N, const BwdScratchView& scr, float* dL_dmean2D,
                         float* dL_dconic, float* dL_dopacity, float* dL_dcolor, float* dL_dsemantic, float* dL_ddepth,
-                        hipStream_t s, bool records) {
+                        hipStream_t s, bool records, uint8_t* contrib) {
     const int rf = bwd_row_floats(sc.S), nch = 4 * ((sc.S + 3) / 4) + 4;
     const ReduceOut out{dL_dmean2D, dL_dconic, dL_dopacity, dL_dcolor, dL_dsemantic, dL_ddepth};
 #define GOI_REDUCE(K)                                                                   \
     do {                                                                                \
-        if (records) launch_reduce_k<K, true>(sc, g, N, nch, scr.rows, scr.flags, scr, out, s);  \
+        if (records) launch_reduce_k<K, true>(sc, g, N, nch, scr.rows, scr.flags, scr, out, s, contrib);  \
         else launch_reduce_k<K, false>(sc, g, N, nch, scr.rows, scr.flags, scr, out, s);         \
     } while (0)
     if (rf == 32) GOI_REDUCE(2);
@@ -261,7 +278,7 @@
     find_big_k<<<dim3((sc.P + 255) / 256), dim3(256), 0, s>>>((uint32_t)N, g.counters + COUNTER_N, order, g.offsets, scr.big_ctl,
                                                              scr.big_desc, (uint32_t)scr.cap_big);
     reduce_big_k<2, true><<<dim3((unsigned)std::min<size_t>(REDUCE_BIG_GRID, scr.cap_big)), dim3(16 * BIG_PARTS), 0, s>>>(
-        scr.big_ctl, scr.big_desc, (uint32_t)scr.cap_big, scr.rows, scr.flags, sc.S, nch, out);
+        scr.big_ctl, scr.big_desc, (uint32_t)scr.cap_big, scr.rows, scr.flags, sc.S, nch, out, nullptr);
 }
 
 void launch_reduce_sem_rows(const GoiRasterScene& sc, const GeomView& g, int N, const BwdScratchView& scr, int row_floats,
diff --git a/goi_hyperplane_amd/csrc/row_sum.h b/goi_hyperplane_amd/csrc/row_sum.h
--- a/goi_hyperplane_amd/csrc/row_sum.h
+++ b/goi_hyperplane_amd/csrc/row_sum.h
@@ -8,7 +8,7 @@
 #endif
 
 template <int K, bool COMPENSATED = false, int INFLIGHT = GOI_REDUCE_INFLIGHT>
-__device__ __forceinline__ void sum_instances(const float* __restrict__ rows, const uint32_t* __restrict__ flags32,
+__device__ __forceinline__ bool sum_instances(const float* __restrict__ rows, const uint32_t* __restrict__ flags32,
                                               size_t inst0, uint32_t cnt, uint32_t w_first, int quarter, int e,
                                               float (&sum)[K], float (&comp)[K]) {
     constexpr int RF = 16 * K;
@@ -17,6 +17,7 @@
 #pragma unroll
     for (int d = 32; d >= 16; d >>= 1) cmax = max(cmax, (uint32_t)__shfl_xor((int)cmax, d, 64));
     uint32_t wq[4] = {w_first, 0u, 0u, 0u};
+    bool any = false;
     if (cmax > 16) {
 #pragma unroll
         for (int sblk = 1; sblk < 4; sblk++) wq[sblk] = load_flags(16u * sblk);
@@ -42,6 +43,7 @@
                 const unsigned long long bal = __ballot(((w >> (8 * q)) & 0xFFu) != 0);
                 m |= ((bal >> (16 * quarter)) & 0xFFFFull) << (16 * q);
             }
+            any |= m != 0;
             const float* chunk = rows + (inst0 + cc) * 4 * RF;
             auto trip = [&](auto nf_c) {
                 constexpr int NF = decltype(nf_c)::value;
@@ -95,6 +97,7 @@
 #pragma unroll
         for (int sblk = 0; sblk < 4; sblk++) wq[sblk] = wn[sblk];
     }
+    return any;
 }
 
 }
diff --git a/goi_hyperplane_amd/csrc/torch_binding.cpp b/goi_hyperplane_amd/csrc/torch_binding.cpp
--- a/goi_hyperplane_amd/csrc/torch_binding.cpp
+++ b/goi_hyperplane_amd/csrc/torch_binding.cpp
@@ -202,7 +202,7 @@
 
 struct PoolEntry {
     Tensor all;
-    Tensor prev_radii;
+    Tensor mask;
     int64_t version;
 };
 struct PoolKey {
@@ -273,7 +273,8 @@
         total += (sizes[i] + 63) / 64 * 64;
     }
     void* stream = stream_of(dev);
-    Tensor flat, prev_radii;
+    Tensor flat, mask;
+    bool mask_valid = false;
     const PoolKey key{(int)dev.index(), stream, total, P, sh_factored ? -M : M, S};
     const bool accumulate = accumulate_into.has_value() && accumulate_into->defined() && P != 0;
     if (accumulate) {
@@ -291,8 +292,9 @@
             for (size_t i = 0; i < v.size(); i++) {
                 if (v[i].all.storage().use_count() != 1 || v[i].all.use_count() != 1) continue;
                 flat = v[i].all;
+                mask = v[i].mask;
                 if ((int64_t)flat._version() == v[i].version) {
-                    prev_radii = v[i].prev_radii;
+                    mask_valid = true;
                     g_pool_hits++;
                 } else {
                     g_pool_dirty++;
@@ -330,20 +332,22 @@
                                      pm, cp, tan_fovx, tan_fovy, false, debug);
         void* scratch = backward_scratch(goi_raster_backward_scratch_bytes(scratch_instances > 0 ? scratch_instances : R, S), dev,
                                          stream, means3D.options().dtype(torch::kByte));
-        const int r = goi_raster_backward3(
+        const bool pooled = g_pool_on && !debug && !accumulate;
+        if (pooled && !mask.defined()) mask = torch::empty({(long long)P}, means3D.options().dtype(torch::kByte));
+        const int r = goi_raster_backward4(
             &sc, R, scratch_instances, accumulate ? GOI_BACKWARD_ACCUMULATE : 0, geomBuffer.data_ptr(), binningBuffer.numel() ? binningBuffer.data_ptr() : nullptr,
             imageBuffer.data_ptr(), rad.data_ptr<int>(), al.p, gc.p, gs.p, gd.p, ga.p, dL_dmeans2D.data_ptr<float>(),
             dL_dconic.data_ptr<float>(), dL_dopacity.data_ptr<float>(), dL_dcolors.data_ptr<float>(),
             dL_dsemantics.data_ptr<float>(), dL_ddepths.data_ptr<float>(), dL_dmeans3D.data_ptr<float>(),
             dL_dcov3D.data_ptr<float>(), dL_dsh.defined() && dL_dsh.numel() ? dL_dsh.data_ptr<float>() : nullptr,
             dL_dscales.data_ptr<float>(), dL_drotations.data_ptr<float>(), scratch,
-            prev_radii.defined() ? prev_radii.data_ptr<int>() : nullptr, stream);
+            nullptr, pooled && mask_valid ? mask.data_ptr<uint8_t>() : nullptr, pooled ? mask.data_ptr<uint8_t>() : nullptr, stream);
         if (r < 0) raise_last();
         std::lock_guard<std::mutex> lk(g_pool_mu);
-        if (g_pool_on && !debug && !accumulate) {
+        if (pooled && g_pool_on) {
             auto& v = g_pool[key];
             if (v.size() >= POOL_BUFFERS_PER_KEY) v.erase(v.begin());
-            v.push_back(PoolEntry{flat, rad, (int64_t)flat._version()});
+            v.push_back(PoolEntry{flat, mask, (int64_t)flat._version()});
         }
     }
     flat = Tensor();
diff --git a/include/goi_raster.h b/include/goi_raster.h
--- a/include/goi_raster.h
+++ b/include/goi_raster.h
@@ -8,7 +8,7 @@
 extern "C" {
 #endif
 
-#define GOI_RASTER_ABI_VERSION 6
+#define GOI_RASTER_ABI_VERSION 7
 
 typedef struct GoiRasterScene {
     int P;
@@ -97,6 +97,16 @@
                          float* dL_dsemantic, float* dL_ddepth, float* dL_dmean3D, float* dL_dcov3D, float* dL_dsh,
                          float* dL_dscale, float* dL_drot, void* scratch, const int* prev_radii, void* stream);
 
+int goi_raster_backward4(const GoiRasterScene* scene, int R, int scratch_instances, int flags, const void* geom_buffer,
+                         const void* binning_buffer, const void* image_buffer, const int* radii, const float* out_alpha,
+                         const float* dL_dout_color, const float* dL_dout_semantic, const float* dL_dout_depth,
+                         const float* dL_dout_alpha, float* dL_dmean2D, float* dL_dconic, float* dL_dopacity, float* dL_dcolor,
+                         float* dL_dsemantic, float* dL_ddepth, float* dL_dmean3D, float* dL_dcov3D, float* dL_dsh,
+                         float* dL_dscale, float* dL_drot, void* scratch, const int* prev_radii, const uint8_t* prev_mask,
+                         uint8_t* row_mask, void* stream);
+
+size_t goi_raster_debug_backward_contrib_offset(int num_rendered, int S);
+
 int goi_raster_backward_semantics(const GoiRasterScene* scene, int R, const void* geom_buffer,
                                   const void* binning_buffer, const void* image_buffer, const int* radii,
                                   const float* out_alpha, const float* dL_dout_semantic, float* dL_dsemantic,
```
